# chaeyeongyun/VQ_SEG

Hardware: AMD Instinct MI355X
Metric: train images/sec @512x512 vqreptunet1x1 K=512 (higher is better)
Workload: dtype bf16; 1 GPU; CPS training iteration (2 x vqreptunet1x1, ResNet-50 encoder, K=[0,0,512,512,512], v1 recipe: 6 forwards + 4 backwards + 2 Adam steps) on 512x512x3 images -- BASELINE configs[2] (the metric's configuration): vqreptunet1x1 512x512, K = 512; labelled_per_gpu=32, unlabelled_per_gpu=32, parallelism=dp1, collectives=none (one process), conv_dtype=bf16

## Files before the change

include/vqseg.h:

```cpp
#ifndef VQSEG_H
#define VQSEG_H

#include <stddef.h>
#include <stdint.h>

#ifdef __cplusplus
extern "C" {
#endif

#define VQSEG_ABI_VERSION 1

#define VQSEG_EINVAL  (-1)
#define VQSEG_ENOSPC  (-2)
#define VQSEG_ENODEV  (-3)

int         vqseg_abi_version(void);
const char* vqseg_last_error(void);
const char* vqseg_kernel_name(const char* entry_point);

int vqseg_set_option(const char* key, int value);

int vqseg_profile_begin(int capacity);
int vqseg_profile_collect(int max_records, int64_t* n_rows_host, int* channels_host,
                          int* n_codes_host, float* ms_host,
                          int* kind_host );

int vqseg_conv_profile_begin(int capacity);
int vqseg_conv_profile_collect(int max_records, double* flops_host, int* kind_host, float* ms_host,
                               int* shape_host );

size_t vqseg_vq_workspace_bytes(int64_t n_rows, int channels, int n_codes);
int vqseg_vq_forward_f32(const float* x, const float* codebook, const void* prepared,
                         int64_t n_rows, int channels, int n_codes, int training,
                         float commitment_weight, float* quant, int64_t* idx, float* loss,
                         float* dead_pct, float* dmin, void* workspace, size_t workspace_bytes,
                         void* stream);

int vqseg_vq_forward_group(int n_levels, int bf16, const void* const* x, const float* const* codebook,
                           const void* const* prepared, const int64_t* n_rows, const int* channels, const int* n_codes,
                           int training, const float* commitment_weight, void* const* quant, int64_t* const* idx,
                           float* const* loss, float* const* dead_pct, void* const* workspace,
                           const size_t* workspace_bytes, void* stream);

size_t vqseg_vq_filter_counter_offset(int64_t n_rows, int channels, int n_codes);

int vqseg_vq_tiles_per_wave(int n_levels, const int64_t* n_rows_host, const int* n_codes_host);

int vqseg_vq_assign_f32(const float* x, const float* codebook, const void* prepared,
                        int64_t n_rows, int channels, int n_codes, int64_t* idx, float* dmin,
                        void* workspace, size_t workspace_bytes, void* stream);
int vqseg_vq_assign_bf16(const void* x, const float* codebook, const void* prepared,
                         int64_t n_rows, int channels, int n_codes, int64_t* idx, float* dmin,
                         void* workspace, size_t workspace_bytes, void* stream);

int vqseg_vq_assign_s3(const void* x, const float* codebook, const void* prepared,
                       int64_t n_rows, int channels, int n_codes, int64_t* idx, float* dmin,
                       void* workspace, size_t workspace_bytes, void* stream);

size_t vqseg_vq_prepared_bytes(int channels, int n_codes);
int vqseg_vq_prepare_f32(const float* codebook, int channels, int n_codes, void* prepared,
                         size_t prepared_bytes, void* stream);

int vqseg_vq_backward_f32(const float* grad_quant, const float* grad_loss, const float* x,
                          const float* quant, int64_t n_rows, int channels,
                          float commitment_weight, float* grad_x, void* stream);

int vqseg_vq_forward_bf16(const void* x, const float* codebook, const void* prepared, int64_t n_rows, int channels,
                          int n_codes, int training, float commitment_weight, void* quant, int64_t* idx, float* loss,
                          float* dead_pct, float* dmin, void* workspace, size_t workspace_bytes, void* stream);
int vqseg_vq_backward_bf16(const void* grad_quant, const float* grad_loss, const void* x, const int64_t* idx,
                           const float* codebook, int64_t n_rows, int channels, float commitment_weight,
                           void* grad_x, void* stream);

size_t vqseg_kmeans_workspace_bytes(int64_t n_rows, int channels, int n_codes);
int vqseg_kmeans_f32(const float* samples, float* means, int64_t* bins, int64_t n_rows,
                     int channels, int n_codes, int iters, void* workspace,
                     size_t workspace_bytes, void* stream);
int vqseg_kmeans_accumulate_f32(const float* samples, const float* means, int64_t n_rows,
                                int channels, int n_codes, float* sums, int64_t* counts,
                                void* workspace, size_t workspace_bytes, void* stream);
int vqseg_kmeans_finalize_f32(const float* sums, const int64_t* counts, float* means,
                              int channels, int n_codes, void* stream);


int vqseg_vq_code_sums(int bf16, const void* x, const int64_t* idx, int64_t n_rows, int channels, int n_codes,
                       float* sums, int64_t* counts, void* workspace, size_t workspace_bytes, void* stream);
int vqseg_vq_ema_update_f32(float* cluster_size, float* embed_avg, float* codebook, const float* sums,
                            const int64_t* counts, int channels, int n_codes, float decay, float eps, float* scratch,
                            void* stream);
int vqseg_vq_revive_candidates(int bf16, const void* x, int64_t n_rows, int channels, int n_codes, uint64_t seed,
                               const int64_t* counter, int rank, int world, float* cand, float* ok, void* stream);
int vqseg_vq_ema_update_revive_f32(float* cluster_size, float* embed_avg, float* codebook, const float* sums,
                                   const int64_t* counts, int channels, int n_codes, float decay, float eps, float* scratch,
                                   const float* cand, const float* ok, float threshold, int64_t* counter, int64_t* revived,
                                   void* stream);


size_t vqseg_conv_packed_elems(int cout, int cin, int kh, int kw, int transpose_flip);
int vqseg_conv_pack_weights_f32(const float* w, int cout, int cin, int kh, int kw, int transpose_flip,
                                void* hi, void* lo, void* stream);

int64_t vqseg_conv_stat_slots(int64_t m_rows, int cout);
int vqseg_conv2d_f(const void* x, const void* x2, int c1, const void* w_hi, const void* w_lo, void* y,
                   float* stat_partial, int n, int h, int w, int cin, int cout, int kh, int kw, int stride,
                   int pad, int reflect, int up, int ho, int wo, int precise, void* stream);

int vqseg_conv2d_affine_f(const void* x, const void* x2, int c1, const void* w_hi, const void* w_lo,
                          const float* scale, const float* shift, const void* res, int relu, void* y,
                          int n, int h, int w, int cin, int cout, int kh, int kw, int stride, int pad, int reflect,
                          int ho, int wo, int precise, void* stream);
int vqseg_conv2d_affine_bits_f(const void* x, const void* w_hi, const float* scale, const float* shift, const void* res,
                               const unsigned char* res_bits, void* y, int n, int h, int w, int cin, int cout, int kh, int kw,
                               int pad, int ho, int wo, void* stream);

size_t vqseg_conv2d_wgrad_workspace_bytes(int n, int h, int w, int cin, int ho, int wo, int cout, int kh, int kw);
int vqseg_conv2d_wgrad_f(const void* gy, const void* x, const void* x2, int c1, int n, int h, int w, int cin,
                         int ho, int wo, int cout, int kh, int kw, int stride, int pad, int reflect, int precise,
                         int cin_out, int im2col, int accumulate, void* workspace, size_t workspace_bytes, float* gw,
                         void* stream);
int vqseg_conv2d_wgrad2_f(const void* gy, const void* x, const void* x2, int n, const void* gy_b, const void* x_b, const void* x2_b,
                          int n_b, int c1, int h, int w, int cin, int ho, int wo, int cout, int kh, int kw, int stride, int pad,
                          int reflect, int precise, int cin_out, int im2col, int accumulate, void* workspace, size_t workspace_bytes,
                          float* gw, void* stream);

int vqseg_bn_sync_ints(int c);
int vqseg_bn_finalize_f(float* partial, int64_t m_rows, int c, const float* gamma, const float* beta,
                        float* run_mean, float* run_var, float momentum, float eps, int training,
                        float* scale, float* shift, float* save_mean, float* save_invstd,
                        int64_t* num_batches_tracked , int* sync, void* stream);
int vqseg_bn_apply_f(int bf16, const void* y, const void* res, const float* scale, const float* shift,
                     int64_t m_rows, int c, int relu, void* out, void* stream);
size_t vqseg_bn_backward_workspace_floats(int64_t m_rows, int c);
int vqseg_bn_backward_f(int bf16, const void* g_out, const void* out, const void* y, const float* mean,
                        const float* invstd, const float* gamma, const float* fwd_scale, const float* fwd_shift,
                        int64_t m_rows, int c, int relu, int training, int accumulate,
                        float* workspace, float* dgamma, float* dbeta, void* g_y, void* g_res, int* sync, void* stream);
int vqseg_bn_apply_bits_f(const void* y, const void* res, const float* scale, const float* shift, int64_t m_rows, int c,
                          void* out, unsigned char* bits, void* stream);
int vqseg_bn_backward_bits_f(const void* g_out, const unsigned char* bits, const void* y, const float* mean,
                             const float* invstd, const float* gamma, int64_t m_rows, int c, int training, int accumulate,
                             float* workspace, float* dgamma, float* dbeta, void* g_y, void* g_res, int* sync, void* stream);

int vqseg_maxpool3x3s2_f(int bf16, int backward, const void* x, const void* g, int n, int h, int w, int c,
                         void* out, unsigned char* idx, void* stream);

int vqseg_bilinear_f(int bf16, int backward, const void* src, int n, int h, int w, int c, int ho, int wo,
                     int align_corners, void* dst, void* stream);

int vqseg_head1x1_forward_f(int bf16, const void* x, const float* w, int64_t m_rows, int cin, int cout,
                            float* y, void* stream);
size_t vqseg_head1x1_backward_workspace_floats(int64_t m_rows, int cin, int cout);
int vqseg_head1x1_backward_f(int bf16, const void* x, const float* w, const float* g, int64_t m_rows, int cin,
                             int cout, void* gx, float* gw, float* workspace, void* stream);
int vqseg_head1x1_backward_add_f(int bf16, const void* x, const float* w, const float* g, int64_t m_rows, int cin,
                                 int cout, void* gx, float* gw, float* workspace, const void* gx_add, void* stream);
int vqseg_maxpool3x3s2_backward_add_f(int bf16, const void* g, const unsigned char* idx, const void* gx_add, int n, int h, int w,
                                      int c, void* gx, void* stream);

int vqseg_im2col_f(int out_bf16, const float* x, int n, int h, int w, int cin, int kh, int kw, int stride,
                   int pad, int reflect, int ho, int wo, int kp, void* out, void* stream);
int vqseg_reflect_fold_f(int bf16, const void* gp, int n, int h, int w, int c, void* gx, void* stream);
int vqseg_stem7_conv_f(int s3, const float* x, const void* w_img, void* y, float* stat_partial, const float* scale, const float* shift, int relu,
                       int n, int h, int w, int reflect, void* stream);
int vqseg_reflect_ring_f(const void* gy, const void* t_hi, void* ring, void* gx, int n, int h, int w, int cgy, int cgx, void* stream);

int vqseg_conv_pack_weights_s3_f32(const float* w, int cout, int cin, int c1, int kh, int kw, void* out, void* stream);

int vqseg_conv_pack_all_f32(const float* w, int cout, int cin, int k, int c1, void* fwd, void* tr, void* s3, void* stream);
size_t vqseg_conv_packed_s2_elems(int cout, int cin, int k);
int vqseg_conv_pack_weights_s2_f32(const float* w, int cout, int cin, int k, void* hi, void* lo, void* stream);
int vqseg_conv2d_dgrad_s2_f(const void* gy, const void* w_hi, const void* w_lo, void* gx, int n, int ho, int wo, int cout, int cin,
                            int k, int oh, int ow, int precise, int accumulate, void* stream);
int64_t vqseg_conv2d_dgrad_s2_fold_rows(int n, int h, int w, int reflect);
int vqseg_conv2d_dgrad_s2_fold_f(const void* gy, const void* w_hi, void* gx, int n, int ho, int wo, int cout, int cin, int h, int w,
                                 int reflect, void* stream);
int vqseg_s3_split_f(const float* x, int64_t rows, int channels, void* y, void* stream);
int vqseg_s3_merge_f(const void* x, int64_t rows, int channels, float* y, void* stream);
int vqseg_s3_maxpool3x3s2_f(const void* x, int n, int h, int w, int c, void* y, void* stream);
int vqseg_s3_bilinear_f(const void* x, int n, int h, int w, int c, int ho, int wo, int align_corners, void* y, void* stream);
int vqseg_cast_f(int to_bf16, const void* x, int64_t n, void* y, void* stream);

size_t vqseg_proto_loss_workspace_bytes(int64_t m_rows, int c, int k);
int vqseg_proto_loss_forward_f(int bf16, const void* x, const float* proto, const int64_t* labels,
                               const unsigned char* keep, const float* conf, int64_t m_rows, int c, int k,
                               int variant, float scale, float margin, int easy_margin,
                               void* workspace, size_t workspace_bytes, double* loss, void* stream);
int vqseg_proto_loss_backward_f(int bf16, const void* x, const float* proto, const int64_t* labels,
                                const unsigned char* keep, const float* conf, int64_t m_rows, int c, int k,
                                int variant, float scale, float margin, int easy_margin, const float* g_loss,
                                void* gx, float* gproto, void* workspace, size_t workspace_bytes, void* stream);

size_t vqseg_dice_workspace_bytes(int b, int c, int64_t hw);
int vqseg_dice_sums_forward_f(const float* logits, int64_t stride_b, int64_t stride_c, int64_t stride_px,
                              const int64_t* target, int b, int c, int64_t hw, int64_t ignore_index,
                              void* workspace, size_t workspace_bytes, float* inter, float* sets, void* stream);
int vqseg_dice_sums_backward_f(const float* logits, int64_t stride_b, int64_t stride_c, int64_t stride_px,
                               const int64_t* target, int b, int c, int64_t hw, int64_t ignore_index,
                               const float* g_inter, const float* g_sets, float* g_logits, void* stream);

int vqseg_dice_ce_sums_forward_f(const float* logits, int64_t stride_b, int64_t stride_c, int64_t stride_px,
                                 const int64_t* target, int b, int c, int64_t hw, int64_t ignore_index,
                                 void* workspace, size_t workspace_bytes, float* inter, float* sets, float* ce,
                                 void* stream);
int vqseg_dice_ce_sums_backward_f(const float* logits, int64_t stride_b, int64_t stride_c, int64_t stride_px,
                                  const int64_t* target, int b, int c, int64_t hw, int64_t ignore_index,
                                  const float* g_inter, const float* g_sets, const float* g_ce, float* g_logits,
                                  void* stream);

int vqseg_softmax_stats_f(const float* logits, int64_t stride_b, int64_t stride_c, int64_t stride_px, int b, int c,
                          int64_t hw, int64_t* label, float* entropy, float* top, void* stream);

int vqseg_confusion_counts_f(const float* logits, int64_t stride_b, int64_t stride_c, int64_t stride_px,
                             const int64_t* target, int b, int c, int64_t hw, int64_t* counts, void* stream);

size_t vqseg_focal_workspace_bytes(int b, int64_t hw);
int vqseg_focal_forward_f(const float* logits, int64_t stride_b, int64_t stride_c, int64_t stride_px,
                          const int64_t* target, int b, int c, int64_t hw, int64_t ignore_index, const float* weight,
                          float alpha, float gamma, int pre_softmax, void* workspace, size_t workspace_bytes,
                          double* per_image, float* loss2, float* loss_map, void* stream);
int vqseg_focal_backward_f(const float* logits, int64_t stride_b, int64_t stride_c, int64_t stride_px,
                           const int64_t* target, int b, int c, int64_t hw, int64_t ignore_index, const float* weight,
                           float alpha, float gamma, int pre_softmax, const float* g_scalar, float scale,
                           const float* g_map, float* g_logits, void* stream);

int vqseg_wce_sums_forward_f(const float* logits, int64_t stride_b, int64_t stride_c, int64_t stride_px,
                             const int64_t* target, int b, int c, int64_t hw, int64_t ignore_index, const float* weight,
                             void* workspace, size_t workspace_bytes, float* ce, void* stream);
int vqseg_wce_sums_backward_f(const float* logits, int64_t stride_b, int64_t stride_c, int64_t stride_px,
                              const int64_t* target, int b, int c, int64_t hw, int64_t ignore_index, const float* weight,
                              const float* g_ce, float* g_logits, void* stream);

int vqseg_class_weight_f(const int64_t* labels, int64_t n, int num_classes, int64_t* counts, float* weight, void* stream);

int vqseg_cps_loss_combine_f(int n_sup, int n_cps, int c, const float* const* inter, const float* const* sets, const float* const* ce,
                             const int* b, float cps_weight, float ce_weight, float eps, const float* const* commit, int n_commit,
                             int levels, float commit_weight, const double* const* proto, int n_proto, float proto_weight,
                             float* const* g_inter, float* const* g_sets, float* const* g_ce, float* out, void* stream);
size_t vqseg_order_stats_workspace_bytes(void);
int vqseg_order_stats_f(const float* x, int64_t n, int64_t k, void* workspace, size_t workspace_bytes, float* out2,
                        void* stream);

#define VQSEG_ADAM_CHUNK 4096
typedef struct VqsegAdamParam {
    float* p;
    const float* g;
    float* m;
    float* v;
    int64_t numel;
    int32_t k, cout, cin, c1;
    void* fwd;
    void* tr;
    void* s3;
} VqsegAdamParam;
int64_t vqseg_adam_work_items(int64_t numel, int k, int cout, int cin);
int vqseg_adam_step_f32(const VqsegAdamParam* params_dev, const int32_t* items_dev, int n_items, double lr, double beta1,
                        double beta2, double eps, int64_t step, void* stream);

typedef struct VqsegEmaParam {
    float* e;
    int32_t copy;
    int32_t reserved;
    void* fwd;
    void* tr;
    void* s3;
} VqsegEmaParam;
int vqseg_adam_ema_step_f32(const VqsegAdamParam* params_dev, const VqsegEmaParam* ema_dev, const int32_t* items_dev, int n_items,
                            double lr, double beta1, double beta2, double eps, int64_t step, double ema_decay, int copy_all,
                            void* stream);

int vqseg_batch_u8_f(int n, const uint8_t* img_cache, const uint8_t* mask_cache, const int64_t* img_offsets_host,
                     const int64_t* mask_offsets_host, int h, int w, int mh, int mw, const float* f32_lut, const int64_t* label_lut,
                     float* img_out, uint8_t* target_out, int64_t* label_out, void* stream);

int vqseg_box_mix_f(int mode, int elem_bytes, const void* src, void* out, int n, int planes, int h, int w, int64_t stride_s,
                    int64_t stride_p, int64_t stride_px, const int32_t* boxes_host, uint64_t fill_bits, void* stream);

int vqseg_affine_warp_f(int mode, int elem_bytes, const void* src, void* out, int n, int planes, int h, int w, int64_t src_stride_s,
                        int64_t out_stride_s, int64_t stride_p, int64_t stride_px, const float* matrices_host, uint64_t fill_bits,
                        void* stream);

int vqseg_resize_argmax_f(const float* const* views_host, const int* flips_host, int n_views, int64_t stride_b, int64_t stride_c,
                          int64_t stride_px, int b, int c, int h, int w, int ho, int wo, uint8_t* label, float* top,
                          const int64_t* target, int64_t* counts, void* stream);

#define VQSEG_BLEND_UNIFORM 0
#define VQSEG_BLEND_LINEAR 1
int vqseg_extract_windows_f(const float* images, int64_t stride_b, int64_t stride_c, int64_t stride_px, int b, int h, int w, int wh, int ww,
                            int sy, int sx, int nh, int nw, const int* flips_host, int n_flips, float* out, void* stream);
int vqseg_merge_argmax_f(const float* const* views_host, const int* flips_host, int n_views, int64_t stride_b, int64_t stride_c,
                         int64_t stride_px, int b, int c, int lh, int lw, int ho, int wo, int wh, int ww, int sy, int sx, int blend,
                         uint8_t* label, float* top, const int64_t* target, int64_t* counts, void* stream);

int vqseg_render_sheet_u8(const float* image, int64_t stride_b, int64_t stride_c, int64_t stride_px, int h, int w, const uint8_t* pred,
                          const int64_t* target, int ht, int wt, int b, int ho, int wo, int c, const int* kinds_host, const int* x0_host,
                          const int* width_host, int n_panels, const float* palette_f_host, const uint8_t* palette_u8_host,
                          const float* fill_f_host, const uint8_t* fill_u8_host, float alpha, int box2, uint8_t* canvas, int64_t pitch,
                          int rows, int cols, void* stream);

size_t vqseg_supcon_workspace_bytes(int64_t hw);
int vqseg_supcon_forward_f(int bf16, const void* f1, const void* f2, int64_t row_stride, int h, int w, int c, const int64_t* gt1,
                           const int64_t* gt2, int ht, int wt, float temperature, void* workspace, size_t workspace_bytes, float* out,
                           void* stream);
int vqseg_supcon_backward_f(int bf16, const void* f1, const void* f2, int64_t row_stride, int h, int w, int c, const int64_t* gt1,
                            const int64_t* gt2, int ht, int wt, float temperature, const float* stats, const float* g_scalar, void* d_f1,
                            void* d_f2, int64_t grad_row_stride, void* stream);

#ifdef __cplusplus
}
#endif
#endif
```

vq_seg_amd/_hip.py:

```python
from __future__ import annotations

import ctypes
import os
from ctypes import c_char_p, c_double, c_float, c_int, c_int64, c_size_t, c_void_p
from typing import Optional, Tuple

import numpy as np
import torch

_HERE = os.path.dirname(os.path.abspath(__file__))
LIB_PATH = os.environ.get("VQSEG_LIB") or os.path.join(_HERE, "libvqseg_hip.so")

SYMBOLS = {
    "vqseg_abi_version": (c_int, []),
    "vqseg_last_error": (c_char_p, []),
    "vqseg_kernel_name": (c_char_p, [c_char_p]),
    "vqseg_set_option": (c_int, [c_char_p, c_int]),
    "vqseg_profile_begin": (c_int, [c_int]),
    "vqseg_profile_collect": (c_int, [c_int, c_void_p, c_void_p, c_void_p, c_void_p, c_void_p]),
    "vqseg_conv_profile_begin": (c_int, [c_int]),
    "vqseg_conv_profile_collect": (c_int, [c_int, c_void_p, c_void_p, c_void_p, c_void_p]),
    "vqseg_vq_workspace_bytes": (c_size_t, [c_int64, c_int, c_int]),
    "vqseg_vq_filter_counter_offset": (c_size_t, [c_int64, c_int, c_int]),
    "vqseg_vq_tiles_per_wave": (c_int, [c_int, c_void_p, c_void_p]),
    "vqseg_vq_forward_f32": (c_int, [c_void_p, c_void_p, c_void_p, c_int64, c_int, c_int, c_int, c_float, c_void_p,
                                     c_void_p, c_void_p, c_void_p, c_void_p, c_void_p, c_size_t, c_void_p]),
    "vqseg_vq_forward_bf16": (c_int, [c_void_p, c_void_p, c_void_p, c_int64, c_int, c_int, c_int, c_float, c_void_p,
                                      c_void_p, c_void_p, c_void_p, c_void_p, c_void_p, c_size_t, c_void_p]),
    "vqseg_vq_forward_group": (c_int, [c_int, c_int] + [c_void_p] * 6 + [c_int, c_void_p] + [c_void_p] * 6 + [c_void_p]),
    "vqseg_vq_backward_bf16": (c_int, [c_void_p, c_void_p, c_void_p, c_void_p, c_void_p, c_int64, c_int, c_float, c_void_p, c_void_p]),
    "vqseg_vq_assign_f32": (c_int, [c_void_p, c_void_p, c_void_p, c_int64, c_int, c_int, c_void_p, c_void_p, c_void_p,
                                    c_size_t, c_void_p]),
    "vqseg_vq_assign_bf16": (c_int, [c_void_p, c_void_p, c_void_p, c_int64, c_int, c_int, c_void_p, c_void_p, c_void_p,
                                     c_size_t, c_void_p]),
    "vqseg_vq_assign_s3": (c_int, [c_void_p, c_void_p, c_void_p, c_int64, c_int, c_int, c_void_p, c_void_p, c_void_p,
                                   c_size_t, c_void_p]),
    "vqseg_vq_prepared_bytes": (c_size_t, [c_int, c_int]),
    "vqseg_vq_prepare_f32": (c_int, [c_void_p, c_int, c_int, c_void_p, c_size_t, c_void_p]),
    "vqseg_vq_backward_f32": (c_int, [c_void_p, c_void_p, c_void_p, c_void_p, c_int64, c_int, c_float, c_void_p,
                                      c_void_p]),
    "vqseg_kmeans_workspace_bytes": (c_size_t, [c_int64, c_int, c_int]),
    "vqseg_kmeans_f32": (c_int, [c_void_p, c_void_p, c_void_p, c_int64, c_int, c_int, c_int, c_void_p, c_size_t,
                                 c_void_p]),
    "vqseg_kmeans_accumulate_f32": (c_int, [c_void_p, c_void_p, c_int64, c_int, c_int, c_void_p, c_void_p, c_void_p,
                                            c_size_t, c_void_p]),
    "vqseg_kmeans_finalize_f32": (c_int, [c_void_p, c_void_p, c_void_p, c_int, c_int, c_void_p]),
    "vqseg_vq_code_sums": (c_int, [c_int, c_void_p, c_void_p, c_int64, c_int, c_int, c_void_p, c_void_p, c_void_p, c_size_t, c_void_p]),
    "vqseg_vq_ema_update_f32": (c_int, [c_void_p, c_void_p, c_void_p, c_void_p, c_void_p, c_int, c_int, c_float, c_float, c_void_p,
                                        c_void_p]),
    "vqseg_vq_revive_candidates": (c_int, [c_int, c_void_p, c_int64, c_int, c_int, ctypes.c_uint64, c_void_p, c_int, c_int, c_void_p, c_void_p,
                                           c_void_p]),
    "vqseg_vq_ema_update_revive_f32": (c_int, [c_void_p, c_void_p, c_void_p, c_void_p, c_void_p, c_int, c_int, c_float, c_float, c_void_p,
                                               c_void_p, c_void_p, c_float, c_void_p, c_void_p, c_void_p]),
    "vqseg_conv_packed_elems": (c_size_t, [c_int] * 5),
    "vqseg_conv_pack_weights_f32": (c_int, [c_void_p] + [c_int] * 5 + [c_void_p, c_void_p, c_void_p]),
    "vqseg_conv_stat_slots": (c_int64, [c_int64, c_int]),
    "vqseg_conv2d_f": (c_int, [c_void_p, c_void_p, c_int, c_void_p, c_void_p, c_void_p, c_void_p] + [c_int] * 14 + [c_void_p]),
    "vqseg_conv2d_affine_f": (c_int, [c_void_p, c_void_p, c_int, c_void_p, c_void_p, c_void_p, c_void_p, c_void_p, c_int, c_void_p] +
                              [c_int] * 13 + [c_void_p]),
    "vqseg_conv2d_wgrad_workspace_bytes": (c_size_t, [c_int] * 9),
    "vqseg_conv2d_wgrad_f": (c_int, [c_void_p, c_void_p, c_void_p] + [c_int] * 17 + [c_void_p, c_size_t, c_void_p, c_void_p]),
    "vqseg_conv2d_wgrad2_f": (c_int, [c_void_p, c_void_p, c_void_p, c_int, c_void_p, c_void_p, c_void_p, c_int] + [c_int] * 16 +
                              [c_void_p, c_size_t, c_void_p, c_void_p]),
    "vqseg_bn_sync_ints": (c_int, [c_int]),
    "vqseg_bn_finalize_f": (c_int, [c_void_p, c_int64, c_int, c_void_p, c_void_p, c_void_p, c_void_p, c_float, c_float, c_int,
                                   c_void_p, c_void_p, c_void_p, c_void_p, c_void_p, c_void_p, c_void_p]),
    "vqseg_bn_apply_f": (c_int, [c_int, c_void_p, c_void_p, c_void_p, c_void_p, c_int64, c_int, c_int, c_void_p, c_void_p]),
    "vqseg_bn_backward_workspace_floats": (c_size_t, [c_int64, c_int]),
    "vqseg_bn_backward_f": (c_int, [c_int] + [c_void_p] * 8 + [c_int64, c_int, c_int, c_int, c_int] + [c_void_p] * 7),
    "vqseg_conv2d_affine_bits_f": (c_int, [c_void_p] * 7 + [c_int] * 10 + [c_void_p]),
    "vqseg_bn_apply_bits_f": (c_int, [c_void_p] * 4 + [c_int64, c_int, c_void_p, c_void_p, c_void_p]),
    "vqseg_bn_backward_bits_f": (c_int, [c_void_p] * 6 + [c_int64, c_int, c_int, c_int] + [c_void_p] * 7),
    "vqseg_maxpool3x3s2_f": (c_int, [c_int, c_int, c_void_p, c_void_p, c_int, c_int, c_int, c_int, c_void_p, c_void_p, c_void_p]),
    "vqseg_bilinear_f": (c_int, [c_int, c_int, c_void_p] + [c_int] * 7 + [c_void_p, c_void_p]),
    "vqseg_head1x1_forward_f": (c_int, [c_int, c_void_p, c_void_p, c_int64, c_int, c_int, c_void_p, c_void_p]),
    "vqseg_head1x1_backward_workspace_floats": (c_size_t, [c_int64, c_int, c_int]),
    "vqseg_head1x1_backward_f": (c_int, [c_int, c_void_p, c_void_p, c_void_p, c_int64, c_int, c_int, c_void_p, c_void_p,
                                        c_void_p, c_void_p]),
    "vqseg_proto_loss_workspace_bytes": (c_size_t, [c_int64, c_int, c_int]),
    "vqseg_proto_loss_forward_f": (c_int, [c_int, c_void_p, c_void_p, c_void_p, c_void_p, c_void_p, c_int64, c_int, c_int, c_int,
                                           c_float, c_float, c_int, c_void_p, c_size_t, c_void_p, c_void_p]),
    "vqseg_proto_loss_backward_f": (c_int, [c_int, c_void_p, c_void_p, c_void_p, c_void_p, c_void_p, c_int64, c_int, c_int, c_int,
                                            c_float, c_float, c_int, c_void_p, c_void_p, c_void_p, c_void_p, c_size_t, c_void_p]),
    "vqseg_dice_workspace_bytes": (c_size_t, [c_int, c_int, c_int64]),
    "vqseg_dice_sums_forward_f": (c_int, [c_void_p, c_int64, c_int64, c_int64, c_void_p, c_int, c_int, c_int64, c_int64, c_void_p, c_size_t,
                                          c_void_p, c_void_p, c_void_p]),
    "vqseg_dice_sums_backward_f": (c_int, [c_void_p, c_int64, c_int64, c_int64, c_void_p, c_int, c_int, c_int64, c_int64, c_void_p,
                                           c_void_p, c_void_p, c_void_p]),
    "vqseg_dice_ce_sums_forward_f": (c_int, [c_void_p, c_int64, c_int64, c_int64, c_void_p, c_int, c_int, c_int64, c_int64, c_void_p,
                                             c_size_t, c_void_p, c_void_p, c_void_p, c_void_p]),
    "vqseg_dice_ce_sums_backward_f": (c_int, [c_void_p, c_int64, c_int64, c_int64, c_void_p, c_int, c_int, c_int64, c_int64, c_void_p,
                                              c_void_p, c_void_p, c_void_p, c_void_p]),
    "vqseg_focal_workspace_bytes": (c_size_t, [c_int, c_int64]),
    "vqseg_focal_forward_f": (c_int, [c_void_p, c_int64, c_int64, c_int64, c_void_p, c_int, c_int, c_int64, c_int64, c_void_p, c_float, c_float,
                                      c_int, c_void_p, c_size_t, c_void_p, c_void_p, c_void_p, c_void_p]),
    "vqseg_focal_backward_f": (c_int, [c_void_p, c_int64, c_int64, c_int64, c_void_p, c_int, c_int, c_int64, c_int64, c_void_p, c_float, c_float,
                                       c_int, c_void_p, c_float, c_void_p, c_void_p, c_void_p]),
    "vqseg_wce_sums_forward_f": (c_int, [c_void_p, c_int64, c_int64, c_int64, c_void_p, c_int, c_int, c_int64, c_int64, c_void_p, c_void_p,
                                         c_size_t, c_void_p, c_void_p]),
    "vqseg_wce_sums_backward_f": (c_int, [c_void_p, c_int64, c_int64, c_int64, c_void_p, c_int, c_int, c_int64, c_int64, c_void_p, c_void_p,
                                          c_void_p, c_void_p]),
    "vqseg_class_weight_f": (c_int, [c_void_p, c_int64, c_int, c_void_p, c_void_p, c_void_p]),
    "vqseg_softmax_stats_f": (c_int, [c_void_p, c_int64, c_int64, c_int64, c_int, c_int, c_int64, c_void_p, c_void_p, c_void_p, c_void_p]),
    "vqseg_confusion_counts_f": (c_int, [c_void_p, c_int64, c_int64, c_int64, c_void_p, c_int, c_int, c_int64, c_void_p, c_void_p]),
    "vqseg_order_stats_workspace_bytes": (c_size_t, []),
    "vqseg_order_stats_f": (c_int, [c_void_p, c_int64, c_int64, c_void_p, c_size_t, c_void_p, c_void_p]),
    "vqseg_im2col_f": (c_int, [c_int, c_void_p] + [c_int] * 12 + [c_void_p, c_void_p]),
    "vqseg_reflect_fold_f": (c_int, [c_int, c_void_p, c_int, c_int, c_int, c_int, c_void_p, c_void_p]),
    "vqseg_reflect_ring_f": (c_int, [c_void_p, c_void_p, c_void_p, c_void_p, c_int, c_int, c_int, c_int, c_int, c_void_p]),
    "vqseg_cast_f": (c_int, [c_int, c_void_p, c_int64, c_void_p, c_void_p]),
    "vqseg_conv_pack_all_f32": (c_int, [c_void_p, c_int, c_int, c_int, c_int, c_void_p, c_void_p, c_void_p, c_void_p]),
    "vqseg_conv_packed_s2_elems": (c_size_t, [c_int, c_int, c_int]),
    "vqseg_conv_pack_weights_s2_f32": (c_int, [c_void_p, c_int, c_int, c_int, c_void_p, c_void_p, c_void_p]),
    "vqseg_conv2d_dgrad_s2_f": (c_int, [c_void_p, c_void_p, c_void_p, c_void_p] + [c_int] * 10 + [c_void_p]),
    "vqseg_stem7_conv_f": (c_int, [c_int, c_void_p, c_void_p, c_void_p, c_void_p, c_void_p, c_void_p] + [c_int] * 5 + [c_void_p]),
    "vqseg_conv2d_dgrad_s2_fold_rows": (ctypes.c_int64, [c_int] * 4),
    "vqseg_cps_loss_combine_f": (c_int, [c_int, c_int, c_int, c_void_p, c_void_p, c_void_p, c_void_p, c_float, c_float, c_float, c_void_p, c_int, c_int,
                                         c_float, c_void_p, c_int, c_float, c_void_p, c_void_p, c_void_p, c_void_p, c_void_p]),
    "vqseg_conv2d_dgrad_s2_fold_f": (c_int, [c_void_p, c_void_p, c_void_p] + [c_int] * 8 + [c_void_p]),
    "vqseg_head1x1_backward_add_f": (c_int, [c_int, c_void_p, c_void_p, c_void_p, c_int64, c_int, c_int, c_void_p, c_void_p,
                                            c_void_p, c_void_p, c_void_p]),
    "vqseg_maxpool3x3s2_backward_add_f": (c_int, [c_int, c_void_p, c_void_p, c_void_p, c_int, c_int, c_int, c_int, c_void_p, c_void_p]),
    "vqseg_conv_pack_weights_s3_f32": (c_int, [c_void_p] + [c_int] * 5 + [c_void_p, c_void_p]),
    "vqseg_s3_split_f": (c_int, [c_void_p, c_int64, c_int, c_void_p, c_void_p]),
    "vqseg_s3_merge_f": (c_int, [c_void_p, c_int64, c_int, c_void_p, c_void_p]),
    "vqseg_s3_maxpool3x3s2_f": (c_int, [c_void_p, c_int, c_int, c_int, c_int, c_void_p, c_void_p]),
    "vqseg_s3_bilinear_f": (c_int, [c_void_p] + [c_int] * 7 + [c_void_p, c_void_p]),
    "vqseg_adam_work_items": (c_int64, [c_int64, c_int, c_int, c_int]),
    "vqseg_adam_step_f32": (c_int, [c_void_p, c_void_p, c_int, c_double, c_double, c_double, c_double, c_int64, c_void_p]),
    "vqseg_adam_ema_step_f32": (c_int, [c_void_p, c_void_p, c_void_p, c_int, c_double, c_double, c_double, c_double, c_int64, c_double, c_int,
                                        c_void_p]),
    "vqseg_batch_u8_f": (c_int, [c_int, c_void_p, c_void_p, c_void_p, c_void_p] + [c_int] * 4 + [c_void_p] * 6),
    "vqseg_box_mix_f": (c_int, [c_int, c_int, c_void_p, c_void_p] + [c_int] * 4 + [c_int64] * 3 + [c_void_p, ctypes.c_uint64, c_void_p]),
    "vqseg_affine_warp_f": (c_int, [c_int, c_int, c_void_p, c_void_p] + [c_int] * 4 + [c_int64] * 4 + [c_void_p, ctypes.c_uint64, c_void_p]),
    "vqseg_resize_argmax_f": (c_int, [c_void_p, c_void_p, c_int] + [c_int64] * 3 + [c_int] * 6 + [c_void_p] * 5),
    "vqseg_extract_windows_f": (c_int, [c_void_p] + [c_int64] * 3 + [c_int] * 9 + [c_void_p, c_int, c_void_p, c_void_p]),
    "vqseg_merge_argmax_f": (c_int, [c_void_p, c_void_p, c_int] + [c_int64] * 3 + [c_int] * 11 + [c_void_p] * 5),
    "vqseg_render_sheet_u8": (c_int, [c_void_p] + [c_int64] * 3 + [c_int] * 2 + [c_void_p] * 2 + [c_int] * 6 + [c_void_p] * 3 + [c_int] +
                              [c_void_p] * 4 + [c_float, c_int, c_void_p, c_int64, c_int, c_int, c_void_p]),
    "vqseg_supcon_workspace_bytes": (c_size_t, [c_int64]),
    "vqseg_supcon_forward_f": (c_int, [c_int, c_void_p, c_void_p, c_int64, c_int, c_int, c_int, c_void_p, c_void_p, c_int, c_int, c_float,
                                       c_void_p, c_size_t, c_void_p, c_void_p]),
    "vqseg_supcon_backward_f": (c_int, [c_int, c_void_p, c_void_p, c_int64, c_int, c_int, c_int, c_void_p, c_void_p, c_int, c_int, c_float,
                                        c_void_p, c_void_p, c_void_p, c_void_p, c_int64, c_void_p]),
}

_lib: Optional[ctypes.CDLL] = None


class HipLibraryError(RuntimeError):
    pass


def _bind_symbols(handle: ctypes.CDLL) -> ctypes.CDLL:
    for name, (res, args) in SYMBOLS.items():
        fn = getattr(handle, name)
        fn.restype, fn.argtypes = res, args
    return handle


def lib() -> ctypes.CDLL:
    global _lib
    if _lib is None:
        if not os.path.exists(LIB_PATH):
            raise HipLibraryError(
                f"{LIB_PATH} not found: build it with `python -c 'import __graft_entry__ as g; g.build()'` "
                f"(or `make -C vq_seg_amd/csrc`). There is no CPU fallback.")
        handle = _bind_symbols(ctypes.CDLL(LIB_PATH))
        if handle.vqseg_abi_version() != 1:
            raise HipLibraryError("libvqseg_hip.so ABI version mismatch")
        for kv in filter(None, os.environ.get("VQSEG_OPTS", "").split(",")):
            key, _, val = kv.partition("=")
            if key.strip().startswith("py_"):
                PY_OPTS[key.strip()] = int(val)
                continue
            if handle.vqseg_set_option(key.strip().encode(), int(val)) < 0:
                raise HipLibraryError(f"VQSEG_OPTS: unknown option {key!r}")
        _lib = handle
    return _lib


PY_OPTS: dict = {}
FILTER_DIAG = None


_BF_DTYPE = {0: torch.float32, 1: torch.bfloat16, 2: torch.bfloat16}


def tptr(t, name: str, dtype=None, numel: Optional[int] = None, bf: Optional[int] = None, at_least: bool = False, dense: bool = True):
    if t is None:
        return None
    if bf is not None:
        dtype = _BF_DTYPE[bf]
    try:
        if (dtype is None or t.dtype is dtype or (type(dtype) is tuple and t.dtype in dtype)) and t.is_cuda and \
                (numel is None or (t.numel() >= numel if at_least else t.numel() == numel)) and \
                (not dense or t.is_contiguous() or (t.dim() == 4 and t.is_contiguous(memory_format=torch.channels_last))):
            return t.data_ptr()
    except AttributeError:
        pass
    return _tptr_report(t, name, dtype, numel, at_least, dense)


def _tptr_report(t, name, dtype, numel, at_least, dense):
    def bad(msg):
        return HipLibraryError(f"{name}: {msg}")
    if not isinstance(t, torch.Tensor):
        raise bad(f"expected a tensor, got {type(t).__name__}")
    if dtype is not None and (t.dtype not in dtype if isinstance(dtype, tuple) else t.dtype != dtype):
        if dense:
            raise bad(f"expected {dtype}, got {t.dtype}")
        names = " or ".join(str(d).removeprefix("torch.") for d in (dtype if isinstance(dtype, tuple) else (dtype,)))
        raise bad(f"expected a {names} tensor, got {t.dtype}")
    if dense and not t.is_contiguous() and not (t.dim() == 4 and t.is_contiguous(memory_format=torch.channels_last)):
        raise bad(f"expected a dense (contiguous) tensor, got strides {tuple(t.stride())} for shape {tuple(t.shape)}")
    if numel is not None and (t.numel() < numel if at_least else t.numel() != numel):
        raise bad(f"the sizes passed along need {'at least ' if at_least else ''}{numel} elements, the tensor has {t.numel()} (shape {tuple(t.shape)})")
    if not t.is_cuda:
        return _NotOnGpu(f"{name}: the HIP path needs a tensor on a 'cuda' (ROCm) device; got {t.device}. There is no CPU fallback.")
    return t.data_ptr()


class _NotOnGpu:
    __slots__ = ("msg",)

    def __init__(self, msg: str):
        self.msg = msg

    def __add__(self, _offset):
        return self


def on_gpu(ptr):
    if type(ptr) is _NotOnGpu:
        raise HipLibraryError(ptr.msg)
    return ptr


def _dev(t: torch.Tensor, dtype: torch.dtype, name: str, numel: Optional[int] = None):
    if t is None:
        raise HipLibraryError(f"{name}: expected a tensor, got None")
    return tptr(t, name, dtype=dtype, numel=numel)


def _stream() -> int:
    return torch.cuda.current_stream().cuda_stream


def _failed(L, name: str, rc: int) -> HipLibraryError:
    return HipLibraryError(f"{name} failed (code {rc}): {L.vqseg_last_error().decode(errors='replace')}")


def launch(name: str, dev, *args, handle=None) -> None:
    L = handle or lib()
    if type(dev) is not torch.device:
        dev = torch.device(dev)
    if dev.type == "cuda":
        try:
            with torch.cuda.device(dev):
                rc = getattr(L, name)(*args, _stream())
        except ctypes.ArgumentError:
            for a in args:
                on_gpu(a)
            raise
        if rc != 0:
            raise _failed(L, name, rc)
        return
    for a in args:
        on_gpu(a)
    raise HipLibraryError(f"{name}: the HIP path needs tensors on a 'cuda' (ROCm) device; got {dev}. There is no CPU fallback.")


def _workspace(nbytes: int, device) -> torch.Tensor:
    return torch.empty(int(nbytes), dtype=torch.uint8, device=device)


def vq_prepare(codebook: torch.Tensor) -> torch.Tensor:
    L = lib()
    k, c = codebook.shape
    wp = _dev(codebook, torch.float32, "codebook")
    nbytes = L.vqseg_vq_prepared_bytes(c, k)
    blob = _workspace(nbytes, codebook.device)
    launch("vqseg_vq_prepare_f32", codebook.device, wp, c, k, blob.data_ptr(), nbytes)
    return blob


def vq_forward(rows: torch.Tensor, codebook: torch.Tensor, training: bool, commitment_weight: float,
               want_dmin: bool = False, prepared: Optional[torch.Tensor] = None):
    L = lib()
    n, c = rows.shape
    k = codebook.shape[0]
    bf16 = rows.dtype == torch.bfloat16
    xp, wp = tptr(rows, "rows", bf=int(bf16), numel=n * c), _dev(codebook, torch.float32, "codebook", k * c)
    dev = rows.device
    quant = torch.empty_like(rows)
    idx = torch.empty(n, dtype=torch.int64, device=dev)
    scal = torch.empty(2, dtype=torch.float32, device=dev)
    dmin = torch.empty(n, dtype=torch.float32, device=dev) if want_dmin else None
    nbytes = L.vqseg_vq_workspace_bytes(n, c, k)
    ws = _workspace(nbytes, dev)
    launch("vqseg_vq_forward_bf16" if bf16 else "vqseg_vq_forward_f32", dev, xp, wp,
           tptr(prepared, "prepared codebook", dtype=torch.uint8, numel=L.vqseg_vq_prepared_bytes(c, k)), n, c, k,
           int(bool(training)), float(commitment_weight), quant.data_ptr(), idx.data_ptr(), scal.data_ptr(), scal.data_ptr() + 4,
           dmin.data_ptr() if want_dmin else None, ws.data_ptr(), nbytes)
    out = (quant, idx, scal[0:1], scal[1])
    return out + (dmin,) if want_dmin else out


def bind(path: str) -> ctypes.CDLL:
    return _bind_symbols(ctypes.CDLL(path))


def vq_forward_group(rows_list, codebooks, prepared_list, training: bool, commitment_weights, handle=None, s3: bool = False):
    L = handle or lib()
    nl = len(rows_list)
    bf16 = 2 if s3 else int(rows_list[0].dtype == torch.bfloat16)
    if s3 and training:
        raise HipLibraryError("vq_forward_group: split-3 rows are an eval-mode format (training must be False)")
    dev = rows_list[0].device
    ptr = lambda ps: (c_void_p * nl)(*map(on_gpu, ps))
    ns = np.array([r.shape[0] for r in rows_list], dtype=np.int64)
    cs = np.array([w.shape[1] for w in codebooks], dtype=np.int32)
    ks = np.array([w.shape[0] for w in codebooks], dtype=np.int32)
    cw = np.array([float(w) for w in commitment_weights], dtype=np.float32)
    xs, wps, preps, quants, idxs, scals, wss = [], [], [], [], [], [], []
    for r, w in zip(rows_list, codebooks):
        if r.dtype != rows_list[0].dtype:
            raise HipLibraryError("vq_forward_group: one row type per call")
        if w.dim() != 2 or r.dim() != 2 or r.shape[1] != (2 if s3 else 1) * w.shape[1]:
            raise HipLibraryError(f"vq_forward_group: rows {tuple(r.shape)} do not match a codebook {tuple(w.shape)}" + (" (split-3 rows: 2C columns)" if s3 else ""))
        xs.append(tptr(r, "rows", bf=bf16, numel=r.shape[0] * r.shape[1]))
        wps.append(_dev(w, torch.float32, "codebook", w.shape[0] * w.shape[1]))
        quants.append(torch.empty_like(r))
        idxs.append(torch.empty(r.shape[0], dtype=torch.int64, device=dev))
        scals.append(torch.empty(2, dtype=torch.float32, device=dev))
        wss.append(_workspace(L.vqseg_vq_workspace_bytes(r.shape[0], w.shape[1], w.shape[0]), dev))
    for w, p_ in zip(codebooks, prepared_list):
        preps.append(tptr(p_, "prepared codebook", dtype=torch.uint8, numel=L.vqseg_vq_prepared_bytes(w.shape[1], w.shape[0])))
    wsb = (c_size_t * nl)(*[w.numel() for w in wss])
    launch("vqseg_vq_forward_group", dev, nl, bf16, ptr(xs), ptr(wps), ptr(preps), ns.ctypes.data, cs.ctypes.data, ks.ctypes.data,
           int(bool(training)), cw.ctypes.data, ptr(q.data_ptr() for q in quants), ptr(i.data_ptr() for i in idxs),
           ptr(s.data_ptr() for s in scals), ptr(s.data_ptr() + 4 for s in scals), ptr(w.data_ptr() for w in wss),
           ctypes.cast(wsb, c_void_p), handle=handle)
    if FILTER_DIAG is not None and bf16:
        for r, w, ws_ in zip(rows_list, codebooks, wss):
            off = L.vqseg_vq_filter_counter_offset(r.shape[0], w.shape[1], w.shape[0])
            FILTER_DIAG.append((r.shape[0], w.shape[1], w.shape[0], ws_[off:off + 256].view(torch.int32) if off else None))
    return [(q, i, s[0:1], s[1]) for q, i, s in zip(quants, idxs, scals)]


def set_option(key: str, value: int) -> int:
    prev = lib().vqseg_set_option(key.encode(), int(value))
    if prev < 0:
        raise HipLibraryError(f"vqseg_set_option: unknown option {key!r} or bad value {value}")
    return prev


def vq_tiles_per_wave(n_rows, n_codes) -> int:
    rows = [n_rows] if isinstance(n_rows, int) else list(n_rows)
    codes = [n_codes] if isinstance(n_codes, int) else list(n_codes)
    if len(rows) != len(codes):
        raise ValueError("vq_tiles_per_wave: one code count per row count")
    t = lib().vqseg_vq_tiles_per_wave(len(rows), (ctypes.c_int64 * len(rows))(*rows), (c_int * len(codes))(*codes))
    if t < 0:
        raise _failed(lib(), "vqseg_vq_tiles_per_wave", t)
    return t


def vq_assign(rows: torch.Tensor, codebook: torch.Tensor, want_dmin: bool = False,
              prepared: Optional[torch.Tensor] = None, want_filter_count: bool = False, s3: bool = False, want_filter_state: bool = False):
    L = lib()
    n, c = rows.shape
    k = codebook.shape[0]
    bf16 = rows.dtype == torch.bfloat16
    if s3:
        if c != 2 * codebook.shape[1]:
            raise HipLibraryError(f"vq_assign: split-3 rows {tuple(rows.shape)} do not match a codebook {tuple(codebook.shape)} (2C columns)")
        c //= 2
    xp, wp = tptr(rows, "rows", bf=2 if s3 else int(bf16), numel=n * c * (2 if s3 else 1)), _dev(codebook, torch.float32, "codebook", k * c)
    dev = rows.device
    idx = torch.empty(n, dtype=torch.int64, device=dev)
    dmin = torch.empty(n, dtype=torch.float32, device=dev) if want_dmin else None
    nbytes = L.vqseg_vq_workspace_bytes(n, c, k)
    ws = _workspace(nbytes, dev)
    launch("vqseg_vq_assign_s3" if s3 else "vqseg_vq_assign_bf16" if bf16 else "vqseg_vq_assign_f32", dev, xp, wp,
           tptr(prepared, "prepared codebook", dtype=torch.uint8, numel=L.vqseg_vq_prepared_bytes(c, k)), n, c, k,
           idx.data_ptr(), dmin.data_ptr() if want_dmin else None, ws.data_ptr(), nbytes)
    if want_filter_count:
        off = L.vqseg_vq_filter_counter_offset(n, c, k) if bf16 else 0
        amb = ws[off:off + 256].view(torch.int32).sum() if off else None
        return (idx, dmin, amb) if want_dmin else (idx, amb)
    if want_filter_state:
        off = L.vqseg_vq_filter_counter_offset(n, c, k) if bf16 else 0
        state = ws[off:off + 260].view(torch.int32).clone() if off else None
        return (idx, dmin, state) if want_dmin else (idx, state)
    return (idx, dmin) if want_dmin else idx


def vq_backward(grad_quant: torch.Tensor, grad_loss: Optional[torch.Tensor], rows: torch.Tensor, quant: torch.Tensor,
                commitment_weight: float) -> torch.Tensor:
    n, c = rows.shape
    gq = _dev(grad_quant, torch.float32, "grad_quant", n * c)
    gl = _dev(grad_loss, torch.float32, "grad_loss", 1) if grad_loss is not None else None
    gx = torch.empty_like(rows)
    launch("vqseg_vq_backward_f32", rows.device, gq, gl, _dev(rows, torch.float32, "rows", n * c), _dev(quant, torch.float32, "quant", n * c),
           n, c, float(commitment_weight), gx.data_ptr())
    return gx


def vq_backward_bf16(grad_quant: torch.Tensor, grad_loss: Optional[torch.Tensor], rows: torch.Tensor, idx: torch.Tensor,
                     codebook: torch.Tensor, commitment_weight: float) -> torch.Tensor:
    n, c = rows.shape
    gq = _dev(grad_quant, torch.bfloat16, "grad_quant", n * c)
    gl = _dev(grad_loss, torch.float32, "grad_loss", 1) if grad_loss is not None else None
    gx = torch.empty_like(rows)
    if codebook.dim() != 2 or codebook.shape[1] != c:
        raise HipLibraryError(f"codebook: expected (K, {c}), got {tuple(codebook.shape)}")
    launch("vqseg_vq_backward_bf16", rows.device, gq, gl, _dev(rows, torch.bfloat16, "rows", n * c), _dev(idx, torch.int64, "idx", n),
           _dev(codebook, torch.float32, "codebook"), n, c, float(commitment_weight), gx.data_ptr())
    return gx


def kmeans(samples: torch.Tensor, means: torch.Tensor, iters: int) -> Tuple[torch.Tensor, torch.Tensor]:
    L = lib()
    n, c = samples.shape
    k = means.shape[0]
    sp, mp = _dev(samples, torch.float32, "samples", n * c), _dev(means, torch.float32, "means", k * c)
    bins = torch.zeros(k, dtype=torch.int64, device=samples.device)
    nbytes = L.vqseg_kmeans_workspace_bytes(n, c, k)
    ws = _workspace(nbytes, samples.device)
    launch("vqseg_kmeans_f32", samples.device, sp, mp, bins.data_ptr(), n, c, k, int(iters), ws.data_ptr(), nbytes)
    return means, bins


def kmeans_accumulate(samples: torch.Tensor, means: torch.Tensor) -> Tuple[torch.Tensor, torch.Tensor]:
    L = lib()
    n, c = samples.shape
    k = means.shape[0]
    sp, mp = _dev(samples, torch.float32, "samples", n * c), _dev(means, torch.float32, "means", k * c)
    sums = torch.empty(k, c, dtype=torch.float32, device=samples.device)
    counts = torch.empty(k, dtype=torch.int64, device=samples.device)
    nbytes = L.vqseg_kmeans_workspace_bytes(n, c, k)
    ws = _workspace(nbytes, samples.device)
    launch("vqseg_kmeans_accumulate_f32", samples.device, sp, mp, n, c, k, sums.data_ptr(), counts.data_ptr(), ws.data_ptr(), nbytes)
    return sums, counts


def kmeans_finalize(sums: torch.Tensor, counts: torch.Tensor, means: torch.Tensor) -> torch.Tensor:
    k, c = means.shape
    launch("vqseg_kmeans_finalize_f32", means.device, _dev(sums, torch.float32, "sums", k * c), _dev(counts, torch.int64, "counts", k),
           _dev(means, torch.float32, "means", k * c), c, k)
    return means


def vq_code_sums(rows: torch.Tensor, idx: torch.Tensor, k: int, out: Optional[torch.Tensor] = None) -> Tuple[torch.Tensor, torch.Tensor]:
    L = lib()
    n, c = rows.shape
    if rows.dtype not in (torch.float32, torch.bfloat16):
        raise HipLibraryError(f"rows: expected torch.float32 or torch.bfloat16, got {rows.dtype}")
    ip = _dev(idx, torch.int64, "idx", n)
    sums = torch.empty(k, c, dtype=torch.float32, device=rows.device) if out is None else out
    counts = torch.empty(k, dtype=torch.int64, device=rows.device)
    nbytes = L.vqseg_kmeans_workspace_bytes(n, c, k)
    ws = _workspace(nbytes, rows.device)
    bf = int(rows.dtype == torch.bfloat16)
    launch("vqseg_vq_code_sums", rows.device, bf, tptr(rows, "rows", bf=bf, numel=n * c), ip, n, c, k,
           sums.data_ptr() if out is None else _dev(out, torch.float32, "out", k * c), counts.data_ptr(), ws.data_ptr(), nbytes)
    return sums, counts


def vq_revive_candidates(rows: torch.Tensor, seed: int, counter: torch.Tensor, k: int, rank: int, world: int, out=None):
    n, c = rows.shape
    if rows.dtype not in (torch.float32, torch.bfloat16):
        raise HipLibraryError(f"rows: expected torch.float32 or torch.bfloat16, got {rows.dtype}")
    bf = int(rows.dtype == torch.bfloat16)
    xp, tp = tptr(rows, "rows", bf=bf, numel=n * c), _dev(counter, torch.int64, "counter", 1)
    if out is None:
        out = (torch.empty(k, c, dtype=torch.float32, device=rows.device), torch.empty(k, dtype=torch.float32, device=rows.device))
    cand, ok = out
    launch("vqseg_vq_revive_candidates", rows.device, bf, xp, n, c, k, int(seed) & 0xFFFFFFFFFFFFFFFF, tp, int(rank), int(world),
           _dev(cand, torch.float32, "candidates", k * c), _dev(ok, torch.float32, "ok", k))
    return cand, ok


def vq_ema_update(cluster_size: torch.Tensor, embed_avg: torch.Tensor, codebook: torch.Tensor, sums: torch.Tensor,
                  counts: torch.Tensor, decay: float, eps: float, candidates: Optional[torch.Tensor] = None,
                  ok: Optional[torch.Tensor] = None, threshold: float = 0.0, counter: Optional[torch.Tensor] = None,
                  revived: Optional[torch.Tensor] = None) -> None:
    k, c = codebook.shape
    if cluster_size.shape != (k,) or embed_avg.shape != (k, c) or sums.shape != (k, c) or counts.shape != (k,):
        raise ValueError("vq_ema_update: shapes must be (K,), (K, C), (K, C), (K, C), (K,)")
    if threshold == 0:
        scratch = torch.empty(1, dtype=torch.float32, device=codebook.device)
        launch("vqseg_vq_ema_update_f32", codebook.device, _dev(cluster_size, torch.float32, "cluster_size"),
               _dev(embed_avg, torch.float32, "embed_avg"), _dev(codebook, torch.float32, "codebook"), _dev(sums, torch.float32, "sums"),
               _dev(counts, torch.int64, "counts"), c, k, float(decay), float(eps), scratch.data_ptr())
        return
    scratch = torch.empty(1 + k, dtype=torch.float32, device=codebook.device)
    launch("vqseg_vq_ema_update_revive_f32", codebook.device, _dev(cluster_size, torch.float32, "cluster_size"),
           _dev(embed_avg, torch.float32, "embed_avg"), _dev(codebook, torch.float32, "codebook"), _dev(sums, torch.float32, "sums"),
           _dev(counts, torch.int64, "counts"), c, k, float(decay), float(eps), scratch.data_ptr(),
           _dev(candidates, torch.float32, "candidates", k * c), _dev(ok, torch.float32, "ok", k), float(threshold),
           _dev(counter, torch.int64, "counter", 1), _dev(revived, torch.int64, "revived", 1))


def batch_u8(img_cache: torch.Tensor, img_offsets, hw: Tuple[int, int], f32_lut: torch.Tensor, img_out: torch.Tensor,
             mask_cache: Optional[torch.Tensor] = None, mask_offsets=None, mask_hw: Tuple[int, int] = (0, 0),
             label_lut: Optional[torch.Tensor] = None, target_out: Optional[torch.Tensor] = None,
             label_out: Optional[torch.Tensor] = None) -> None:
    n = len(img_offsets)
    (h, w), (mh, mw) = hw, mask_hw
    io = np.ascontiguousarray(img_offsets, dtype=np.int64)
    mo = np.ascontiguousarray(mask_offsets, dtype=np.int64) if mask_offsets is not None else None
    if n and (int(io.min()) < 0 or int(io.max()) + h * w * 3 > img_cache.numel()):
        raise HipLibraryError("batch_u8: an image offset lies outside the image cache")
    if mask_cache is not None:
        if mo is None or len(mo) != n:
            raise HipLibraryError("batch_u8: one mask offset per sample required")
        if n and (int(mo.min()) < 0 or int(mo.max()) + mh * mw > mask_cache.numel()):
            raise HipLibraryError("batch_u8: a mask offset lies outside the mask cache")
    if img_out.dim() != 4 or not img_out.is_contiguous(memory_format=torch.channels_last):
        raise HipLibraryError("batch_u8: img_out must be a channels_last (n, 3, h, w) tensor")
    launch("vqseg_batch_u8_f", img_out.device, n, tptr(img_cache, "img_cache", dtype=torch.uint8), tptr(mask_cache, "mask_cache", dtype=torch.uint8),
           io.ctypes.data, mo.ctypes.data if mo is not None else None, h, w, mh, mw,
           tptr(f32_lut, "f32_lut", dtype=torch.float32, numel=256), tptr(label_lut, "label_lut", dtype=torch.int64, numel=256),
           tptr(img_out, "img_out", dtype=torch.float32, numel=n * 3 * h * w),
           tptr(target_out, "target_out", dtype=torch.uint8, numel=n * mh * mw),
           tptr(label_out, "label_out", dtype=torch.int64, numel=n * mh * mw))


BOX_MIX_DTYPES = (torch.uint8, torch.bfloat16, torch.float32, torch.int64)
BOX_MIX_CALLS = 0


def box_mix(src: torch.Tensor, boxes, mode: str = "mix", fill=0, out: Optional[torch.Tensor] = None) -> torch.Tensor:
    global BOX_MIX_CALLS
    if mode not in ("mix", "fill"):
        raise HipLibraryError(f"box_mix: mode must be 'mix' or 'fill', got {mode!r}")
    if not isinstance(src, torch.Tensor) or src.dim() not in (3, 4):
        raise HipLibraryError("box_mix: src must be a (n, P, h, w) or (n, h, w) tensor")
    n, (h, w) = src.shape[0], src.shape[-2:]
    planes = src.shape[1] if src.dim() == 4 else 1
    bx = np.ascontiguousarray(boxes, dtype=np.int32)
    if bx.shape != (n, 4):
        raise HipLibraryError(f"box_mix: one (y1, x1, cut_h, cut_w) box per sample required: {n} samples, boxes of shape {bx.shape}")
    if n and (int(bx.min()) < 0 or int((bx[:, 0] + bx[:, 2]).max()) > h or int((bx[:, 1] + bx[:, 3]).max()) > w):
        raise HipLibraryError(f"box_mix: a box lies outside the {h} x {w} image")
    if out is None:
        out = torch.empty_like(src)
    elif not isinstance(out, torch.Tensor) or out.shape != src.shape or out.stride() != src.stride():
        raise HipLibraryError("box_mix: out must have src's shape and layout")
    numel = n * planes * h * w
    sp, op = tptr(src, "src", dtype=BOX_MIX_DTYPES, numel=numel), tptr(out, "out", dtype=src.dtype, numel=numel)
    if numel == 0:
        raise HipLibraryError("box_mix: empty tensor")
    strides = (planes * h * w, h * w, 1) if src.is_contiguous() else (planes * h * w, 1, planes)
    bits = int.from_bytes(torch.tensor([fill], dtype=src.dtype).view(torch.uint8).numpy().tobytes(), "little") if mode == "fill" else 0
    launch("vqseg_box_mix_f", src.device, int(mode == "fill"), src.element_size(), sp, op, n, planes, h, w, *strides, bx.ctypes.data, bits)
    BOX_MIX_CALLS += 1
    return out


AFFINE_WARP_BILINEAR_DTYPES = (torch.float32, torch.bfloat16)
AFFINE_WARP_NEAREST_DTYPES = (torch.uint8, torch.int8, torch.bool, torch.int16, torch.bfloat16, torch.float16, torch.int32, torch.float32, torch.int64,
                              torch.float64)
AFFINE_WARP_CALLS = 0


def affine_warp(src: torch.Tensor, matrices, mode: str = "bilinear", fill=0, out: Optional[torch.Tensor] = None) -> torch.Tensor:
    global AFFINE_WARP_CALLS
    if mode not in ("bilinear", "nearest"):
        raise HipLibraryError(f"affine_warp: mode must be 'bilinear' or 'nearest', got {mode!r}")
    if not isinstance(src, torch.Tensor) or src.dim() not in (3, 4):
        raise HipLibraryError("affine_warp: src must be a (n, P, h, w) or (n, h, w) tensor")
    n, (h, w) = src.shape[0], src.shape[-2:]
    planes = src.shape[1] if src.dim() == 4 else 1
    try:
        mats = np.ascontiguousarray(matrices, dtype=np.float32)
    except (TypeError, ValueError):
        raise HipLibraryError("affine_warp: matrices must be n rows of six numbers") from None
    if mats.shape != (n, 6):
        raise HipLibraryError(f"affine_warp: one (M00, M01, 0, M10, M11, 0) row per sample required: {n} samples, matrices of shape {mats.shape}")
    if not np.isfinite(mats).all():
        raise HipLibraryError("affine_warp: a matrix entry is not finite")
    if mats[:, (2, 5)].any():
        raise HipLibraryError("affine_warp: the translation slots (entries 2 and 5 of a row) are reserved and must be 0")
    dtypes = AFFINE_WARP_BILINEAR_DTYPES if mode == "bilinear" else AFFINE_WARP_NEAREST_DTYPES
    numel = n * planes * h * w
    sp = tptr(src, "src", dtype=dtypes, numel=numel)
    if numel == 0:
        raise HipLibraryError("affine_warp: empty tensor")
    planar = src.is_contiguous()
    inner = (h * w, 1) if planar else (1, planes)
    out_stride = planes * h * w
    if out is None:
        out = torch.empty_like(src)
        op = tptr(out, "out", dtype=src.dtype, numel=numel)
    else:
        if not isinstance(out, torch.Tensor) or out.shape != src.shape:
            raise HipLibraryError("affine_warp: out must have src's shape and layout")
        one = out[:1]
        if (one.is_contiguous() if planar else (one.dim() == 4 and one.is_contiguous(memory_format=torch.channels_last))) and \
                (n == 1 or out.stride(0) >= out_stride):
            out_stride = out.stride(0) if n > 1 else out_stride
        else:
            raise HipLibraryError("affine_warp: out must have src's shape and layout")
        op = tptr(out, "out", dtype=src.dtype, numel=numel, dense=False)
        if type(sp) is int and type(op) is int and sp == op:
            raise HipLibraryError("affine_warp: out of place only")
    bits = int.from_bytes(torch.tensor([fill], dtype=src.dtype).view(torch.uint8).numpy().tobytes(), "little") if mode == "nearest" else 0
    launch("vqseg_affine_warp_f", src.device, int(mode == "nearest"), src.element_size(), sp, op, n, planes, h, w, planes * h * w, out_stride,
           *inner, mats.ctypes.data, bits)
    AFFINE_WARP_CALLS += 1
    return out


RENDER_KINDS = {"image": 0, "target": 1, "pred": 2, "detail": 3, "mix_pred": 4, "mix_detail": 5, "fill": 6}
RENDER_SHEET_CALLS = 0


def render_sheet(canvas: torch.Tensor, panels, size, num_classes: int, palette, fill=(1.0, 1.0, 1.0), image: Optional[torch.Tensor] = None,
                 pred: Optional[torch.Tensor] = None, target: Optional[torch.Tensor] = None, alpha: float = 0.4, box2: bool = False,
                 cols: Optional[int] = None) -> torch.Tensor:
    global RENDER_SHEET_CALLS
    E = HipLibraryError
    b, ho, wo = (int(v) for v in size)
    c = int(num_classes)
    rows = b * ho
    if not isinstance(canvas, torch.Tensor) or canvas.dim() != 3 or canvas.shape[2] != 3:
        raise E("render_sheet: canvas must be a (rows, cols, 3) uint8 tensor")
    orows, ocols = int(canvas.shape[0]), int(canvas.shape[1])
    cols = ocols * (2 if box2 else 1) if cols is None else int(cols)
    if box2 and (rows % 2 or cols % 2):
        raise E(f"render_sheet: box2 needs a sheet of even height and width, got {rows} x {cols}")
    if (orows, ocols) != ((rows // 2, cols // 2) if box2 else (rows, cols)):
        raise E(f"render_sheet: a {rows} x {cols} sheet{' halved by box2' if box2 else ''} needs a canvas of "
                f"{(rows // 2, cols // 2) if box2 else (rows, cols)} pixels, got {(orows, ocols)}")
    if orows == 0 or ocols == 0:
        raise E("render_sheet: empty canvas")
    if canvas.stride(2) != 1 or (ocols > 1 and canvas.stride(1) != 3) or (orows > 1 and canvas.stride(0) < 3 * ocols):
        raise E(f"render_sheet: canvas pixels must be dense RGB bytes with rows at least a row apart, got strides {tuple(canvas.stride())}")
    pitch = canvas.stride(0) if orows > 1 else 3 * ocols
    rows_ = [(RENDER_KINDS.get(k, -1) if isinstance(k, str) else int(k), int(x), int(wd)) for k, x, wd in panels]
    if any(k < 0 for k, _, _ in rows_):
        raise E(f"render_sheet: panel kinds are {sorted(RENDER_KINDS)}, got {[p[0] for p in panels]}")
    pal = np.ascontiguousarray(palette, dtype=np.float64)
    if pal.shape != (2 * c + 1, 3):
        raise E(f"render_sheet: the palette of {c} classes has {2 * c + 1} rows of 3 (class, wrong, ignore), got shape {pal.shape}")
    fil = np.ascontiguousarray(fill, dtype=np.float64).reshape(-1)
    if fil.shape != (3,):
        raise E("render_sheet: fill is one RGB colour")
    pal_f, fil_f = pal.astype(np.float32), fil.astype(np.float32)
    pal_u, fil_u = (np.floor(np.clip(a, 0.0, 1.0) * 255.0).astype(np.uint8) for a in (pal, fil))
    ip = pp = tp = None
    strides, (h, w), (ht, wt) = (0, 0, 0), (0, 0), (0, 0)
    if image is not None:
        if not isinstance(image, torch.Tensor) or image.dim() != 4 or image.shape[0] != b or image.shape[1] != 3:
            raise E(f"render_sheet: image must be a ({b}, 3, h, w) tensor")
        h, w = int(image.shape[2]), int(image.shape[3])
        ip = tptr(image, "image", dtype=torch.float32, numel=b * 3 * h * w)
        strides = (3 * h * w, h * w, 1) if image.is_contiguous() else (3 * h * w, 1, 3)
    if pred is not None:
        if not isinstance(pred, torch.Tensor) or tuple(pred.shape) != (b, ho, wo):
            raise E(f"render_sheet: pred must have the shape {(b, ho, wo)}, got {tuple(getattr(pred, 'shape', ()))}")
        pp = tptr(pred, "pred", dtype=torch.uint8, numel=b * ho * wo)
    if target is not None:
        if not isinstance(target, torch.Tensor) or target.dim() != 3 or target.shape[0] != b:
            raise E(f"render_sheet: target must be a ({b}, ht, wt) tensor")
        ht, wt = int(target.shape[1]), int(target.shape[2])
        tp = tptr(target, "target", dtype=torch.int64, numel=b * ht * wt)
    cp = tptr(canvas, "canvas", dtype=torch.uint8, numel=orows * ocols * 3, dense=False)
    arr = np.ascontiguousarray(rows_, dtype=np.int32).reshape(-1, 3).T.copy()
    launch("vqseg_render_sheet_u8", canvas.device, ip, *strides, h, w, pp, tp, ht, wt, b, ho, wo, c, arr[0].ctypes.data, arr[1].ctypes.data,
           arr[2].ctypes.data, len(rows_), pal_f.ctypes.data, pal_u.ctypes.data, fil_f.ctypes.data, fil_u.ctypes.data, float(alpha), int(bool(box2)),
           cp, pitch, rows, cols)
    RENDER_SHEET_CALLS += 1
    return canvas


def _checked(name: str, *args, counts: bool = False) -> int:
    rc = getattr(lib(), name)(*args)
    if rc < 0 or (rc and not counts):
        raise _failed(lib(), name, rc)
    return rc


def profile_begin(capacity: int = 4096) -> None:
    _checked("vqseg_profile_begin", int(capacity))


def conv_profile_begin(capacity: int = 65536) -> None:
    _checked("vqseg_conv_profile_begin", int(capacity))


def conv_profile_collect(capacity: int = 65536, with_shape: bool = False):
    fl = np.zeros(capacity, dtype=np.float64)
    kd = np.zeros(capacity, dtype=np.int32)
    ms = np.zeros(capacity, dtype=np.float32)
    sh = np.zeros((capacity, 4), dtype=np.int32)
    cnt = _checked("vqseg_conv_profile_collect", capacity, fl.ctypes.data, kd.ctypes.data, ms.ctypes.data, sh.ctypes.data if with_shape else None, counts=True)
    if with_shape:
        return [(float(fl[i]), int(kd[i]), float(ms[i]), tuple(int(v) for v in sh[i])) for i in range(cnt)]
    return [(float(fl[i]), int(kd[i]), float(ms[i])) for i in range(cnt)]


def profile_collect(capacity: int = 4096, with_kind: bool = False):
    n = np.zeros(capacity, dtype=np.int64)
    c = np.zeros(capacity, dtype=np.int32)
    k = np.zeros(capacity, dtype=np.int32)
    ms = np.zeros(capacity, dtype=np.float32)
    kd = np.zeros(capacity, dtype=np.int32)
    cnt = _checked("vqseg_profile_collect", capacity, n.ctypes.data, c.ctypes.data, k.ctypes.data, ms.ctypes.data, kd.ctypes.data, counts=True)
    if with_kind:
        return [(int(n[i]), int(c[i]), int(k[i]), float(ms[i]), int(kd[i])) for i in range(cnt)]
    return [(int(n[i]), int(c[i]), int(k[i]), float(ms[i])) for i in range(cnt)]
```

vq_seg_amd/csrc/vq_host.hip:

```cpp
#include <hip/hip_runtime.h>
#include <stdint.h>

#include <vector>

#include "options.h"
#include "vq_internal.h"

namespace vqseg {

static inline int round_up(int v, int m) { return (v + m - 1) / m * m; }

static inline size_t up256(size_t v) { return (v + 255) & ~(size_t)255; }

static bool filter_shape_ok(int C, int K) { return K % 256 == 0 && C % 32 == 0 && K <= 65536; }

PreparedLayout prepared_layout(int C, int K) {
    const int Kp = round_up(K, 32);
    PreparedLayout l;
    l.off_e4 = 0;
    l.off_enorm = (size_t)C * Kp * sizeof(float);
    l.off_enmax = up256(l.off_enorm + (size_t)Kp * sizeof(float));
    l.off_eb = l.off_enmax + 256;
    l.bytes = filter_shape_ok(C, K) ? up256(l.off_eb + (size_t)2 * C * Kp * sizeof(unsigned short)) : l.off_eb;
    return l;
}

PreparedView prepared_view(const void* prepared, int C, int K) {
    const PreparedLayout l = prepared_layout(C, K);
    char* base = const_cast<char*>(static_cast<const char*>(prepared));
    return {reinterpret_cast<float*>(base + l.off_e4), reinterpret_cast<float*>(base + l.off_enorm),
            reinterpret_cast<float*>(base + l.off_enmax), reinterpret_cast<unsigned short*>(base + l.off_eb)};
}

size_t prepared_bytes(int C, int K) { return prepared_layout(C, K).bytes; }

static int g_vq_max_tiles = 8;
static int g_vq_fine_split = 1;
static int g_vq_bf16_filter = 1;
static int g_vq_filter_force_all = 0;
static int g_vq_filter_launches = 0;
static int g_vq_s3_filter = 1;
static const Option VQ_OPTIONS[] = {
    {"vq_max_tiles_per_wave", &g_vq_max_tiles, OPT_POW2_FAIL, 1, 8},
    {"vq_fine_split", &g_vq_fine_split, OPT_FLAG},
    {"vq_bf16_filter", &g_vq_bf16_filter, OPT_FLAG},
    {"vq_filter_force_all", &g_vq_filter_force_all, OPT_FLAG},
    {"vq_filter_launches", &g_vq_filter_launches},
    {"vq_s3_filter", &g_vq_s3_filter, OPT_FLAG},
};

int vq_set_option(const char* key, int value) { return apply_option(VQ_OPTIONS, key, value); }

VqPlan vq_plan(int64_t N, int C, int K) {
    VqPlan p;
    p.Cp = C;
    p.Kp = round_up(K, 32);
    size_t off = 0;
    p.off_prepared = off;
    off += prepared_bytes(C, K);
    p.off_keys = off;
    off += up256((size_t)N * sizeof(unsigned long long));
    p.off_hist = off;
    off += up256((size_t)p.Kp * sizeof(int));
    p.off_partial = off;
    off += (size_t)GATHER_BLOCKS_MAX * sizeof(float);
    off = up256(off);
    p.off_summary = p.off_brow = p.off_amb = p.off_pair_rc = off;
    p.pair_cap = 0;
    if (filter_shape_ok(C, K)) {
        p.off_summary = off;
        off += up256((size_t)N * (p.Kp / F_SUB) * sizeof(unsigned long long));
        p.off_brow = off;
        off += up256((size_t)N * sizeof(float));
        p.off_amb = off;
        off += 512;
        const long total_cap = 4 * N < (1L << 30) ? 4 * N : (1L << 30);
        p.pair_cap = (int)((total_cap + F_LISTS - 1) / F_LISTS);
        if (p.pair_cap < 1024) p.pair_cap = 1024;
        p.off_pair_rc = off;
        off += up256((size_t)p.pair_cap * F_LISTS * sizeof(unsigned long long));
    }
    p.bytes = up256(off);
    long blocks = (N + GATHER_ROWS_PER_BLOCK - 1) / GATHER_ROWS_PER_BLOCK;
    p.gather_blocks = (int)(blocks < GATHER_BLOCKS_MAX ? (blocks > 0 ? blocks : 1) : GATHER_BLOCKS_MAX);
    const int k1 = K;
    p.T = vq_group_tiles(1, &N, &k1);
    return p;
}

hipError_t launch_prepare(const float* W, int K, int C, void* prepared, hipStream_t st) {
    const int Kp = round_up(K, 32);
    const PreparedView pv = prepared_view(prepared, C, K);
    launch_prepare_exact(W, K, C, Kp, pv.E4, pv.enorm, st);
    if (filter_shape_ok(C, K)) launch_prepare_filter(W, K, C, Kp, pv.enorm, pv.Eb, pv.en_max, st);
    return hipGetLastError();
}

struct ProfShape {
    int64_t n;
    int c, k;
    int slot, group;
    int kind;
};
struct Profile {
    bool enabled = false;
    int capacity = 0;
    std::vector<hipEvent_t> ev;
    std::vector<ProfShape> shape;
};
static Profile g_prof;

hipError_t profile_begin(int capacity) {
    profile_release();
    g_prof.ev.resize((size_t)capacity * 2);
    for (auto& e : g_prof.ev) {
        hipError_t rc = hipEventCreate(&e);
        if (rc != hipSuccess) return rc;
    }
    g_prof.shape.clear();
    g_prof.capacity = capacity;
    g_prof.enabled = true;
    return hipSuccess;
}

void profile_release() {
    for (auto& e : g_prof.ev) (void)hipEventDestroy(e);
    g_prof.ev.clear();
    g_prof.shape.clear();
    g_prof.enabled = false;
    g_prof.capacity = 0;
}

int profile_collect(int max_records, int64_t* n, int* c, int* k, float* ms, int* kind) {
    g_prof.enabled = false;
    const int cnt = (int)g_prof.shape.size();
    int out = 0;
    for (int i = 0; i < cnt && out < max_records; ++i) {
        const ProfShape& sh = g_prof.shape[i];
        if (hipEventSynchronize(g_prof.ev[2 * sh.slot + 1]) != hipSuccess) break;
        float t = 0.f;
        if (hipEventElapsedTime(&t, g_prof.ev[2 * sh.slot], g_prof.ev[2 * sh.slot + 1]) != hipSuccess) break;
        double mine = 2.0 * (double)sh.n * sh.c * sh.k, all = 0.0;
        for (int j = sh.slot; j < sh.slot + sh.group && j < cnt; ++j) all += 2.0 * (double)g_prof.shape[j].n * g_prof.shape[j].c * g_prof.shape[j].k;
        n[out] = sh.n;
        c[out] = sh.c;
        k[out] = sh.k;
        ms[out] = (float)(t * (all > 0 ? mine / all : 1.0));
        if (kind) kind[out] = sh.kind;
        ++out;
    }
    profile_release();
    return out;
}


static unsigned assign_workgroups(int64_t N, int Kp, int T) {
    const long row_tiles = (N + ROWS_PER_WG - 1) / ROWS_PER_WG;
    return (unsigned)((row_tiles + 7) / 8 * 8 * (Kp / (32 * T)));
}

constexpr long VQ_FINE_WGS = 4096;
static long vq_group_wgs(int n, const int64_t* N, const int* K, int t) {
    long wgs = 0;
    for (int i = 0; i < n; ++i) {
        const int tiles = round_up(K[i], 32) / 32;
        if (tiles % t) return -1;
        wgs += ((N[i] + ROWS_PER_WG - 1) / ROWS_PER_WG) * (tiles / t);
    }
    return wgs;
}
int vq_group_tiles(int n, const int64_t* N, const int* K) {
    if (g_vq_fine_split)
        for (int t = g_vq_max_tiles; t >= 4; t >>= 1)
            if (vq_group_wgs(n, N, K, t) >= VQ_FINE_WGS) return t;
    for (int t = g_vq_max_tiles; t >= 1; t >>= 1) {
        const long wgs = vq_group_wgs(n, N, K, t);
        if (wgs >= 0 && (wgs >= 512 || t == 1)) return t;
    }
    return 1;
}

hipError_t launch_assign_group(int n, const void* const* x, int x_bf16, const int64_t* N, const int* C, const int* K,
                               const void* const* prepared, const VqPlan* plans, char* const* ws, int64_t* const* idx,
                               float* const* dmin, int T, hipStream_t st, const float* const* codebooks) {
    if (n < 1 || n > VQ_MAX_LEVELS) return hipErrorInvalidValue;
    int order[VQ_MAX_LEVELS];
    for (int i = 0; i < n; ++i) order[i] = i;
    for (int i = 0; i < n; ++i)
        for (int j = i + 1; j < n; ++j)
            if (C[order[j]] > C[order[i]]) { const int t = order[i]; order[i] = order[j]; order[j] = t; }
    bool filter = x_bf16 == VQ_ROWS_S3 ? g_vq_s3_filter != 0 : (x_bf16 && g_vq_bf16_filter);
    for (int i = 0; i < n; ++i) filter = filter && filter_shape_ok(C[i], K[i]);
    VqLevel lv[VQ_MAX_LEVELS];
    VqFilterGroup fg;
    fg.n = n;
    unsigned end = 0, fend = 0, rend = 0, send = 0, iend = 0;
    VqInitGroup ig;
    ig.n = n;
    for (int q = 0; q < n; ++q) {
        const int i = order[q];
        const PreparedView pv = prepared_view(prepared[i], C[i], K[i]);
        unsigned long long* keys = reinterpret_cast<unsigned long long*>(ws[i] + plans[i].off_keys);
        {
            long ib = (N[i] + 4095) / 4096;
            ib = ib < 1 ? 1 : (ib > 256 ? 256 : ib);
            iend += (unsigned)ib;
            ig.lv[q] = VqInitLevel{keys, (long)N[i], nullptr, reinterpret_cast<int*>(ws[i] + plans[i].off_hist), plans[i].Kp, iend};
        }
        end += assign_workgroups(N[i], plans[i].Kp, T);
        lv[q] = VqLevel{x[i], pv.E4, pv.enorm, keys, (long)N[i], C[i], plans[i].Kp, end};
        lv[q].K = K[i];
        if (filter) {
            int* amb = reinterpret_cast<int*>(ws[i] + plans[i].off_amb);
            ig.lv[q].amb = amb;
            lv[q].gate = amb + F_LISTS;
            lv[q].gate_cap = 0;
            const long row_tiles = (N[i] + F_ROWS - 1) / F_ROWS;
            fend += (unsigned)((row_tiles + 7) / 8 * 8 * (plans[i].Kp / F_CODES));
            rend += (unsigned)((N[i] + 255) / 256);
            {
                long per = (N[i] / 256 + F_LISTS - 1) / F_LISTS;
                if (per < 4) per = 4;
                if (per > 16) per = 16;
                send += (unsigned)(per * F_LISTS);
            }
            fg.lv[q] = VqFilterLevel{x[i], pv.Eb, pv.enorm, pv.en_max,
                                     reinterpret_cast<unsigned long long*>(ws[i] + plans[i].off_summary),
                                     reinterpret_cast<float*>(ws[i] + plans[i].off_brow),
                                     reinterpret_cast<unsigned long long*>(ws[i] + plans[i].off_pair_rc), amb, plans[i].pair_cap, keys,
                                     codebooks ? codebooks[i] : nullptr, pv.E4, (long)N[i], C[i], plans[i].Kp, fend, rend, send};
        }
    }
    launch_group_init(ig, st);
    const bool rec = g_prof.enabled && (int)g_prof.shape.size() + n <= g_prof.capacity;
    const size_t slot = g_prof.shape.size();
    if (rec) {
        for (int i = 0; i < n; ++i) g_prof.shape.push_back({N[i], C[i], K[i], (int)slot, n, filter ? 2 : (x_bf16 == VQ_ROWS_BF16 ? 1 : 0)});
        (void)hipEventRecord(g_prof.ev[2 * slot], st);
    }
    if (filter) {
        ++g_vq_filter_launches;
        launch_filter(fg, x_bf16, g_vq_filter_force_all, st);
    }
    launch_assign_levels(lv, n, T, x_bf16, st);
    if (rec) (void)hipEventRecord(g_prof.ev[2 * slot + 1], st);
    hipError_t e = hipGetLastError();
    if (e != hipSuccess) return e;
    for (int i = 0; i < n; ++i) {
        launch_unpack_level(i, N, K, plans, ws, idx, dmin, st);
        if (filter && dmin && dmin[i]) {
            const PreparedView pv = prepared_view(prepared[i], C[i], K[i]);
            launch_exact_dist(x[i], x_bf16, pv.E4, plans[i].Kp, pv.enorm, idx[i], N[i], C[i], dmin[i], st);
        }
    }
    return hipGetLastError();
}

hipError_t launch_assign(const void* x, int x_bf16, int64_t N, int C, int K, const void* prepared, const VqPlan& p, char* ws,
                         int64_t* idx, float* dmin, hipStream_t st, const float* codebook) {
    return launch_assign_group(1, &x, x_bf16, &N, &C, &K, &prepared, &p, &ws, &idx, &dmin, p.T, st, codebook ? &codebook : nullptr);
}

KmPlan km_plan(int64_t N, int C, int K) {
    KmPlan p;
    p.vq = vq_plan(N, C, K);
    size_t off = p.vq.bytes;
    p.off_idx = off;
    off += (size_t)N * sizeof(int64_t);
    p.off_counts = off;
    off += (size_t)round_up(K + 1, 64) * sizeof(int);
    p.off_offsets = off;
    off += (size_t)round_up(K + 1, 64) * sizeof(int);
    p.off_members = off;
    off += (size_t)N * sizeof(int);
    p.off_sums = off;
    off += (size_t)K * C * sizeof(float);
    p.off_counts64 = off;
    off += (size_t)round_up(K, 32) * sizeof(int64_t);
    p.row_blocks = (int)((N + KM_RB - 1) / KM_RB);
    p.max_segments = (int)(N / KM_SEG + K);
    p.off_hist = off;
    off += (size_t)round_up(p.row_blocks * K, 64) * sizeof(int);
    p.off_segoff = off;
    off += (size_t)round_up(K + 1, 64) * sizeof(int);
    p.off_partial = off;
    off += (size_t)p.max_segments * C * sizeof(float);
    p.bytes = up256(off);
    return p;
}

hipError_t launch_km_accumulate(const float* samples, const float* means, int64_t N, int C, int K, const KmPlan& p,
                                char* ws, float* sums, int64_t* counts64, hipStream_t st) {
    hipError_t e = launch_prepare(means, K, C, ws + p.vq.off_prepared, st);
    if (e != hipSuccess) return e;
    int64_t* idx = reinterpret_cast<int64_t*>(ws + p.off_idx);
    e = launch_assign(samples, 0, N, C, K, ws + p.vq.off_prepared, p.vq, ws, idx, nullptr, st);
    if (e != hipSuccess) return e;
    return launch_code_sums(samples, 0, idx, N, C, K, p, ws, sums, counts64, st);
}

}
```

vq_seg_amd/csrc/vq_internal.h:

```cpp
#pragma once
#include "nn_device.h"
#include "vq_kernels.h"

namespace vqseg {

typedef float f32x16 __attribute__((ext_vector_type(16)));
typedef float f32x4 __attribute__((ext_vector_type(4)));
typedef unsigned int u32x2 __attribute__((ext_vector_type(2)));
typedef unsigned int u32x4 __attribute__((ext_vector_type(4)));

constexpr int ROWS_PER_WG = 128;
constexpr int F_ROWS = 128, F_CODES = 256, F_SUB = 128;
constexpr int F_LISTS = 64;
constexpr int GATHER_BLOCKS_MAX = 2048;
constexpr int GATHER_ROWS_PER_BLOCK = 16;
constexpr int KM_RB = 1024;
constexpr int KM_SEG = 128;

constexpr int VQ_ROWS_F32 = 0, VQ_ROWS_BF16 = 1, VQ_ROWS_S3 = 2;
__device__ __forceinline__ float s3_elem(const unsigned short* row, int C, int c) {
    return __builtin_bit_cast(float, (unsigned)row[c] << 16) + __builtin_bit_cast(float, (unsigned)row[C + c] << 16);
}

struct VqLevel {
    const void* x;
    const float* E4;
    const float* enorm;
    unsigned long long* keys;
    long N;
    int C, Kp;
    unsigned wg_end;
    const int* gate = nullptr;
    int gate_cap = 0;
    int K = 0;
};
struct VqFilterLevel {
    const void* x;
    const unsigned short* Eb;
    const float* enorm;
    const float* en_max;
    unsigned long long* summary;
    float* brow;
    unsigned long long* pair_rc;
    int* pair_count;
    int pair_cap;
    unsigned long long* keys;
    const float* W;
    const float* E4;
    long N;
    int C, Kp;
    unsigned wg_end;
    unsigned rblk_end;
    unsigned sblk_end;
};
struct VqFilterGroup {
    VqFilterLevel lv[VQ_MAX_LEVELS];
    int n;
};
struct VqInitLevel {
    unsigned long long* keys;
    long n;
    int* amb;
    int* hist;
    int kp;
    unsigned end;
};
struct VqInitGroup {
    VqInitLevel lv[VQ_MAX_LEVELS];
    int n;
};

struct PreparedView {
    float* E4;
    float* enorm;
    float* en_max;
    unsigned short* Eb;
};
PreparedView prepared_view(const void* prepared, int C, int K);

void launch_assign_levels(const VqLevel* lv, int n, int T, int row_type, hipStream_t st);
void launch_prepare_filter(const float* W, int K, int C, int Kp, const float* enorm, unsigned short* Eb, float* en_max, hipStream_t st);
void launch_filter(const VqFilterGroup& fg, int row_type, int force_all, hipStream_t st);
void launch_exact_dist(const void* x, int row_type, const float* E4, int Kp, const float* enorm, const int64_t* idx, int64_t N, int C, float* dmin,
                       hipStream_t st);
void launch_group_init(const VqInitGroup& ig, hipStream_t st);
void launch_unpack_level(int i, const int64_t* N, const int* K, const VqPlan* plans, char* const* ws, int64_t* const* idx,
                         float* const* dmin, hipStream_t st);
void launch_prepare_exact(const float* W, int K, int C, int Kp, float* E4, float* enorm, hipStream_t st);

}
```

vq_seg_amd/csrc/vq_kernels.h:

```cpp
#pragma once
#include <hip/hip_runtime.h>
#include <stddef.h>
#include <stdint.h>

namespace vqseg {

constexpr int VQ_MAX_LEVELS = 4;

struct VqPlan {
    int Cp, Kp;
    int T;
    size_t off_prepared, off_keys, off_hist, off_partial, bytes;
    int gather_blocks;
    size_t off_summary, off_brow, off_amb, off_pair_rc;
    int pair_cap;
};
struct PreparedLayout {
    size_t off_e4, off_enorm, off_enmax, off_eb, bytes;
};
PreparedLayout prepared_layout(int C, int K);
int vq_set_option(const char* key, int value);
struct KmPlan {
    VqPlan vq;
    size_t off_idx, off_counts, off_offsets, off_members, off_sums, off_counts64, off_hist, off_segoff, off_partial, bytes;
    int row_blocks, max_segments;
};

hipError_t profile_begin(int capacity);
void profile_release();
int profile_collect(int max_records, int64_t* n, int* c, int* k, float* ms, int* kind);

VqPlan vq_plan(int64_t N, int C, int K);
KmPlan km_plan(int64_t N, int C, int K);

size_t prepared_bytes(int C, int K);
hipError_t launch_prepare(const float* W, int K, int C, void* prepared, hipStream_t st);
hipError_t launch_assign(const void* x, int x_bf16, int64_t N, int C, int K, const void* prepared, const VqPlan& p, char* ws,
                         int64_t* idx, float* dmin, hipStream_t st, const float* codebook = nullptr);
int vq_group_tiles(int n, const int64_t* N, const int* K);
hipError_t launch_assign_group(int n, const void* const* x, int x_bf16, const int64_t* N, const int* C, const int* K,
                               const void* const* prepared, const VqPlan* plans, char* const* ws, int64_t* const* idx,
                               float* const* dmin, int T, hipStream_t st, const float* const* codebooks = nullptr);
hipError_t launch_gather(const void* x, int bf16, const float* W, const int64_t* idx, int64_t N, int C, int K, int training,
                         float cw, const VqPlan& p, char* ws, void* quant, float* loss, float* dead, hipStream_t st);
hipError_t launch_backward(const float* gq, const float* gloss, const float* x, const float* q, int64_t N, int C,
                           float cw, float* gx, hipStream_t st);
hipError_t launch_backward_idx(const void* gq, const float* gloss, const void* x, const int64_t* idx, const float* W, int64_t N,
                               int C, float cw, void* gx, hipStream_t st);
hipError_t launch_km_accumulate(const float* samples, const float* means, int64_t N, int C, int K, const KmPlan& p,
                                char* ws, float* sums, int64_t* counts64, hipStream_t st);
hipError_t launch_code_sums(const void* x, int x_bf16, const int64_t* idx, int64_t N, int C, int K, const KmPlan& p, char* ws,
                            float* sums, int64_t* counts64, hipStream_t st);
hipError_t launch_ema_update(float* cluster_size, float* embed_avg, float* codebook, const float* sums, const int64_t* counts64,
                             int K, int C, float decay, float eps, float* total, hipStream_t st);
hipError_t launch_revive_candidates(const void* x, int x_bf16, int64_t N, int C, int K, uint64_t seed, const int64_t* t, int rank,
                                    int world, float* cand, float* ok, hipStream_t st);
hipError_t launch_ema_update_revive(float* cluster_size, float* embed_avg, float* codebook, const float* sums, const int64_t* counts64,
                                    int K, int C, float decay, float eps, float* scratch, const float* cand, const float* ok,
                                    float threshold, int64_t* t, int64_t* revived, hipStream_t st);
hipError_t launch_km_finalize(const float* sums, const int64_t* counts64, float* means, int C, int K, hipStream_t st);

}
```

vq_seg_amd/csrc/vq_tail.hip:

```cpp
#include <hip/hip_runtime.h>
#include <stdint.h>

#include "vq_internal.h"

namespace vqseg {

static_assert(F_LISTS + 1 <= 128, "the init launch zeroes 128 ints of a level's counter block");
__global__ __launch_bounds__(256) void vq_group_init_kernel(const VqInitGroup g) {
    int q = 0;
    while (q + 1 < g.n && blockIdx.x >= g.lv[q].end) ++q;
    const VqInitLevel& L = g.lv[q];
    const unsigned first = q ? g.lv[q - 1].end : 0u, nb = L.end - first, b = blockIdx.x - first;
    for (long i = (long)b * 256 + threadIdx.x; i < L.n; i += (long)nb * 256) L.keys[i] = ~0ull;
    if (b == 0) {
        if (L.amb && threadIdx.x < 128) L.amb[threadIdx.x] = 0;
        for (int k = threadIdx.x; k < L.kp; k += 256) L.hist[k] = 0;
    }
}

__global__ __launch_bounds__(256) void vq_unpack_keys(const unsigned long long* __restrict__ keys, long N,
                                                      long long* __restrict__ idx, float* __restrict__ dmin,
                                                      int* __restrict__ hist, int K, int lds_hist) {
    extern __shared__ int lh[];
    if (hist && lds_hist)
        for (int k = threadIdx.x; k < K; k += 256) lh[k] = 0;
    __syncthreads();
    for (long i = (long)blockIdx.x * 256 + threadIdx.x; i < N; i += (long)gridDim.x * 256) {
        const unsigned long long k = keys[i];
        unsigned code = (unsigned)(k & 0xffffffffull);
        if (code >= (unsigned)K) code = 0u;
        idx[i] = (long long)code;
        if (dmin) dmin[i] = __uint_as_float((unsigned int)(k >> 32));
        if (hist && code < (unsigned)K) atomicAdd((lds_hist ? lh : hist) + code, 1);
    }
    if (hist && lds_hist) {
        __syncthreads();
        for (int k = threadIdx.x; k < K; k += 256) {
            const int c = lh[k];
            if (c) atomicAdd(hist + k, c);
        }
    }
}

template <typename TA>
__device__ __forceinline__ f32x4 ld4(const TA* p, long v) {
    if constexpr (sizeof(TA) == 4) {
        return reinterpret_cast<const f32x4*>(p)[v];
    } else {
        const u32x2 r = reinterpret_cast<const u32x2*>(p)[v];
        return f32x4{__builtin_bit_cast(float, r[0] << 16), __builtin_bit_cast(float, r[0] & 0xFFFF0000u),
                     __builtin_bit_cast(float, r[1] << 16), __builtin_bit_cast(float, r[1] & 0xFFFF0000u)};
    }
}
template <typename TA>
__device__ __forceinline__ void st4(TA* p, long v, const f32x4& q) {
    if constexpr (sizeof(TA) == 4) {
        reinterpret_cast<f32x4*>(p)[v] = q;
    } else {
        u32x2 r;
#pragma unroll
        for (int e = 0; e < 2; ++e) {
            const __bf16 lo = (__bf16)q[2 * e], hi = (__bf16)q[2 * e + 1];
            r[e] = (unsigned)__builtin_bit_cast(unsigned short, lo) | ((unsigned)__builtin_bit_cast(unsigned short, hi) << 16);
        }
        reinterpret_cast<u32x2*>(p)[v] = r;
    }
}

template <typename TA>
__global__ __launch_bounds__(256) void vq_gather_kernel(const TA* __restrict__ x, const float* __restrict__ W,
                                                        const long long* __restrict__ idx, long N, int C,
                                                        int training, TA* __restrict__ quant,
                                                        float* __restrict__ partial) {
    const int lane = threadIdx.x & 63, wave = threadIdx.x >> 6;
    const int c4 = C >> 2;
    float sq = 0.0f;
    constexpr int RG = 4;
    for (long row0 = ((long)blockIdx.x * 4 + wave) * RG; row0 < N; row0 += (long)gridDim.x * 4 * RG) {
        long long k[RG];
#pragma unroll
        for (int j = 0; j < RG; ++j) k[j] = row0 + j < N ? idx[row0 + j] : 0;
        if constexpr (__is_same(TA, S3Row)) {
            for (int v = lane; v < (C >> 3); v += 64) {
                f32x4 e0[RG], e1[RG];
#pragma unroll
                for (int j = 0; j < RG; ++j)
                    if (row0 + j < N) {
                        e0[j] = reinterpret_cast<const f32x4*>(W + k[j] * (long)C)[2 * v];
                        e1[j] = reinterpret_cast<const f32x4*>(W + k[j] * (long)C)[2 * v + 1];
                    }
#pragma unroll
                for (int j = 0; j < RG; ++j)
                    if (row0 + j < N) {
                        const float q[8] = {e0[j][0], e0[j][1], e0[j][2], e0[j][3], e1[j][0], e1[j][1], e1[j][2], e1[j][3]};
                        s3_store8(reinterpret_cast<unsigned short*>(quant) + (row0 + j) * 2L * C, C, 8 * v, q);
                    }
            }
            continue;
        }
        for (int v = lane; v < c4; v += 64) {
            f32x4 e[RG], xv[RG];
#pragma unroll
            for (int j = 0; j < RG; ++j) {
                if (row0 + j < N) {
                    e[j] = reinterpret_cast<const f32x4*>(W + k[j] * (long)C)[v];
                    if (training) xv[j] = ld4<TA>(x + (row0 + j) * (long)C, v);
                }
            }
#pragma unroll
            for (int j = 0; j < RG; ++j) {
                if (row0 + j < N) {
                    TA* qr = quant + (row0 + j) * (long)C;
                    if (training) {
                        f32x4 q;
#pragma unroll
                        for (int i = 0; i < 4; ++i) {
                            q[i] = xv[j][i] + (e[j][i] - xv[j][i]);
                            const float dlt = q[i] - xv[j][i];
                            sq = __builtin_fmaf(dlt, dlt, sq);
                        }
                        st4<TA>(qr, v, q);
                    } else {
                        st4<TA>(qr, v, e[j]);
                    }
                }
            }
        }
    }
#pragma unroll
    for (int m = 32; m >= 1; m >>= 1) sq += __shfl_xor(sq, m);
    __shared__ float wsum[4];
    if (lane == 0) wsum[wave] = sq;
    __syncthreads();
    if (threadIdx.x == 0) partial[blockIdx.x] = (wsum[0] + wsum[1]) + (wsum[2] + wsum[3]);
}

__global__ __launch_bounds__(256) void vq_finalize_kernel(const float* __restrict__ partial, int n_partial,
                                                          const int* __restrict__ hist, int K, int training,
                                                          float commitment_weight, double numel,
                                                          float* __restrict__ loss, float* __restrict__ dead_pct) {
    __shared__ double sd[256];
    __shared__ int sz[256];
    double s = 0.0;
    for (int i = threadIdx.x; i < n_partial; i += 256) s += (double)partial[i];
    int z = 0;
    for (int k = threadIdx.x; k < K; k += 256) z += (hist[k] == 0);
    sd[threadIdx.x] = s;
    sz[threadIdx.x] = z;
    __syncthreads();
    for (int m = 128; m >= 1; m >>= 1) {
        if (threadIdx.x < m) {
            sd[threadIdx.x] += sd[threadIdx.x + m];
            sz[threadIdx.x] += sz[threadIdx.x + m];
        }
        __syncthreads();
    }
    if (threadIdx.x == 0) {
        float l = 0.0f;
        if (training && commitment_weight > 0.0f) l = (float)(sd[0] / numel) * commitment_weight;
        loss[0] = l;
        dead_pct[0] = 100.0f * ((float)sz[0] / (float)K);
    }
}

__global__ __launch_bounds__(256) void vq_backward_kernel(const float* __restrict__ gq, const float* __restrict__ gloss,
                                                          const float* __restrict__ x, const float* __restrict__ q,
                                                          long n4, float coef, float* __restrict__ gx) {
    const float k = gloss ? gloss[0] * coef : 0.0f;
    for (long i = (long)blockIdx.x * 256 + threadIdx.x; i < n4; i += (long)gridDim.x * 256) {
        const f32x4 g = reinterpret_cast<const f32x4*>(gq)[i];
        const f32x4 xv = reinterpret_cast<const f32x4*>(x)[i];
        const f32x4 qv = reinterpret_cast<const f32x4*>(q)[i];
        f32x4 o;
#pragma unroll
        for (int j = 0; j < 4; ++j) o[j] = __builtin_fmaf(k, xv[j] - qv[j], g[j]);
        reinterpret_cast<f32x4*>(gx)[i] = o;
    }
}

__global__ __launch_bounds__(256) void vq_backward_idx_kernel(const __bf16* __restrict__ gq, const float* __restrict__ gloss,
                                                              const __bf16* __restrict__ x, const long long* __restrict__ idx,
                                                              const float* __restrict__ W, long N, int C, float coef,
                                                              __bf16* __restrict__ gx) {
    const float k = gloss ? gloss[0] * coef : 0.0f;
    const int c4 = C >> 2;
    const long n4 = N * c4;
    for (long i = (long)blockIdx.x * 256 + threadIdx.x; i < n4; i += (long)gridDim.x * 256) {
        const long row = i / c4;
        const int v = (int)(i - row * c4);
        const f32x4 g = ld4<__bf16>(gq, i), xv = ld4<__bf16>(x, i);
        const f32x4 e = reinterpret_cast<const f32x4*>(W + idx[row] * (long)C)[v];
        f32x4 o;
#pragma unroll
        for (int j = 0; j < 4; ++j) o[j] = __builtin_fmaf(k, xv[j] - e[j], g[j]);
        st4<__bf16>(gx, i, o);
    }
}

void launch_group_init(const VqInitGroup& ig, hipStream_t st) {
    hipLaunchKernelGGL(vq_group_init_kernel, dim3(ig.lv[ig.n - 1].end), dim3(256), 0, st, ig);
}

void launch_unpack_level(int i, const int64_t* N, const int* K, const VqPlan* plans, char* const* ws, int64_t* const* idx,
                         float* const* dmin, hipStream_t st) {
    int* hist = reinterpret_cast<int*>(ws[i] + plans[i].off_hist);
    long blocks = (N[i] + 1023) / 1024;
    if (blocks > 512) blocks = 512;
    if (blocks < 1) blocks = 1;
    const int lds_hist = K[i] <= 8192;
    hipLaunchKernelGGL(vq_unpack_keys, dim3((unsigned)blocks), dim3(256), lds_hist ? (size_t)K[i] * sizeof(int) : 0, st,
                       reinterpret_cast<unsigned long long*>(ws[i] + plans[i].off_keys), (long)N[i],
                       reinterpret_cast<long long*>(idx[i]), dmin ? dmin[i] : nullptr, hist, K[i], lds_hist);
}

hipError_t launch_gather(const void* x, int bf16, const float* W, const int64_t* idx, int64_t N, int C, int K, int training,
                         float cw, const VqPlan& p, char* ws, void* quant, float* loss, float* dead, hipStream_t st) {
    int* hist = reinterpret_cast<int*>(ws + p.off_hist);
    float* partial = reinterpret_cast<float*>(ws + p.off_partial);
    if (bf16 == VQ_ROWS_S3)
        hipLaunchKernelGGL(vq_gather_kernel<S3Row>, dim3(p.gather_blocks), dim3(256), 0, st, static_cast<const S3Row*>(x), W,
                           reinterpret_cast<const long long*>(idx), (long)N, C, 0, static_cast<S3Row*>(quant), partial);
    else if (bf16)
        hipLaunchKernelGGL(vq_gather_kernel<__bf16>, dim3(p.gather_blocks), dim3(256), 0, st, static_cast<const __bf16*>(x), W,
                           reinterpret_cast<const long long*>(idx), (long)N, C, training, static_cast<__bf16*>(quant), partial);
    else
        hipLaunchKernelGGL(vq_gather_kernel<float>, dim3(p.gather_blocks), dim3(256), 0, st, static_cast<const float*>(x), W,
                           reinterpret_cast<const long long*>(idx), (long)N, C, training, static_cast<float*>(quant), partial);
    hipLaunchKernelGGL(vq_finalize_kernel, dim3(1), dim3(256), 0, st, partial, p.gather_blocks, hist, K, training, cw,
                       (double)N * (double)C, loss, dead);
    return hipGetLastError();
}

hipError_t launch_backward(const float* gq, const float* gloss, const float* x, const float* q, int64_t N, int C,
                           float cw, float* gx, hipStream_t st) {
    const long n4 = (long)N * C / 4;
    const float coef = (float)((double)cw * 2.0 / ((double)N * (double)C));
    long blocks = (n4 + 255) / 256;
    if (blocks > 4096) blocks = 4096;
    if (blocks < 1) blocks = 1;
    hipLaunchKernelGGL(vq_backward_kernel, dim3((unsigned)blocks), dim3(256), 0, st, gq, gloss, x, q, n4, coef, gx);
    return hipGetLastError();
}

hipError_t launch_backward_idx(const void* gq, const float* gloss, const void* x, const int64_t* idx, const float* W, int64_t N,
                               int C, float cw, void* gx, hipStream_t st) {
    const long n4 = (long)N * C / 4;
    const float coef = (float)((double)cw * 2.0 / ((double)N * (double)C));
    long blocks = (n4 + 255) / 256;
    if (blocks > 4096) blocks = 4096;
    if (blocks < 1) blocks = 1;
    hipLaunchKernelGGL(vq_backward_idx_kernel, dim3((unsigned)blocks), dim3(256), 0, st, static_cast<const __bf16*>(gq), gloss,
                       static_cast<const __bf16*>(x), reinterpret_cast<const long long*>(idx), W, (long)N, C, coef,
                       static_cast<__bf16*>(gx));
    return hipGetLastError();
}

}
```

vq_seg_amd/csrc/vqseg_abi.hip:

```cpp
#include <hip/hip_runtime.h>
#include <stdarg.h>
#include <stdio.h>
#include <string.h>

#include "../../include/vqseg.h"
#include "vq_kernels.h"

namespace {
thread_local char g_err[512] = "";

int fail(int code, const char* fmt, ...) {
    va_list ap;
    va_start(ap, fmt);
    vsnprintf(g_err, sizeof(g_err), fmt, ap);
    va_end(ap);
    return code;
}
int hip_fail(hipError_t e, const char* where) {
    snprintf(g_err, sizeof(g_err), "%s: %s", where, hipGetErrorString(e));
    return (int)e;
}
bool aligned16(const void* p) { return (reinterpret_cast<uintptr_t>(p) & 15u) == 0; }

int check_shape(int64_t n, int c, int k) {
    if (n <= 0 || c <= 0 || k <= 0) return fail(VQSEG_EINVAL, "n_rows, channels and n_codes must be positive (got %lld, %d, %d)", (long long)n, c, k);
    if (c % 4) return fail(VQSEG_EINVAL, "channels must be a multiple of 4 (got %d)", c);
    if (n > (int64_t)1 << 31) return fail(VQSEG_EINVAL, "n_rows too large (%lld)", (long long)n);
    return 0;
}
}

extern "C" {

int vqseg_set_error(int code, const char* msg) {
    snprintf(g_err, sizeof(g_err), "%s", msg);
    return code;
}

int vqseg_abi_version(void) { return VQSEG_ABI_VERSION; }
const char* vqseg_last_error(void) { return g_err; }

const char* vqseg_kernel_name(const char* entry) {
    if (!entry) return "";
    if (!strcmp(entry, "vqseg_vq_forward_f32") || !strcmp(entry, "vqseg_vq_assign_f32") ||
        !strcmp(entry, "vqseg_kmeans_f32") || !strcmp(entry, "vqseg_kmeans_accumulate_f32"))
        return "vq_assign_f32_kernel";
    if (!strcmp(entry, "vqseg_vq_backward_f32")) return "vq_backward_kernel";
    if (!strcmp(entry, "vqseg_kmeans_finalize_f32")) return "km_finalize_kernel";
    return "";
}

int vqseg_profile_begin(int capacity) {
    if (capacity <= 0 || capacity > (1 << 20)) return fail(VQSEG_EINVAL, "capacity out of range");
    hipError_t e = vqseg::profile_begin(capacity);
    if (e != hipSuccess) return hip_fail(e, "profile_begin");
    return 0;
}

int vqseg_profile_collect(int max_records, int64_t* n_rows_host, int* channels_host, int* n_codes_host, float* ms_host, int* kind_host) {
    if (max_records <= 0 || !n_rows_host || !channels_host || !n_codes_host || !ms_host)
        return fail(VQSEG_EINVAL, "bad argument");
    return vqseg::profile_collect(max_records, n_rows_host, channels_host, n_codes_host, ms_host, kind_host);
}

size_t vqseg_vq_workspace_bytes(int64_t n, int c, int k) {
    if (n <= 0 || c <= 0 || k <= 0) return 0;
    return vqseg::vq_plan(n, c, k).bytes;
}

size_t vqseg_vq_filter_counter_offset(int64_t n, int c, int k) {
    if (n <= 0 || c <= 0 || k <= 0) return 0;
    const vqseg::VqPlan p = vqseg::vq_plan(n, c, k);
    return p.off_amb == p.off_summary ? 0 : p.off_amb;
}

int vqseg_vq_tiles_per_wave(int n_levels, const int64_t* n_rows_host, const int* n_codes_host) {
    if (n_levels < 1 || n_levels > vqseg::VQ_MAX_LEVELS || !n_rows_host || !n_codes_host) return fail(VQSEG_EINVAL, "tiles_per_wave: bad argument");
    for (int i = 0; i < n_levels; ++i)
        if (n_rows_host[i] <= 0 || n_codes_host[i] <= 0) return fail(VQSEG_EINVAL, "tiles_per_wave: non-positive size");
    return vqseg::vq_group_tiles(n_levels, n_rows_host, n_codes_host);
}

size_t vqseg_vq_prepared_bytes(int c, int k) {
    if (c <= 0 || k <= 0) return 0;
    return vqseg::prepared_bytes(c, k);
}

int vqseg_vq_prepare_f32(const float* codebook, int c, int k, void* prepared, size_t prepared_bytes, void* stream) {
    if (int rc = check_shape(1, c, k)) return rc;
    if (!codebook || !prepared) return fail(VQSEG_EINVAL, "null pointer argument");
    if (!aligned16(codebook) || !aligned16(prepared)) return fail(VQSEG_EINVAL, "codebook and prepared must be 16-byte aligned");
    if (prepared_bytes < vqseg::prepared_bytes(c, k))
        return fail(VQSEG_ENOSPC, "prepared buffer %zu < %zu bytes", prepared_bytes, vqseg::prepared_bytes(c, k));
    hipError_t e = vqseg::launch_prepare(codebook, k, c, prepared, static_cast<hipStream_t>(stream));
    if (e != hipSuccess) return hip_fail(e, "vq codebook prepare");
    return 0;
}

static int vq_assign_any(const void* x, int x_bf16, const float* codebook, const void* prepared, int64_t n, int c, int k,
                         int64_t* idx, float* dmin, void* ws, size_t ws_bytes, void* stream) {
    if (int rc = check_shape(n, c, k)) return rc;
    if (x_bf16 && c % 8) return fail(VQSEG_EINVAL, "%s rows need channels %% 8 == 0", x_bf16 == 2 ? "split-3" : "bf16");
    if (!x || !idx || !ws || (!codebook && !prepared)) return fail(VQSEG_EINVAL, "null pointer argument");
    if (!aligned16(x) || !aligned16(ws) || !aligned16(prepared) || !aligned16(codebook))
        return fail(VQSEG_EINVAL, "x, codebook, prepared and workspace must be 16-byte aligned");
    const vqseg::VqPlan p = vqseg::vq_plan(n, c, k);
    if (ws_bytes < p.bytes) return fail(VQSEG_ENOSPC, "workspace %zu < %zu bytes", ws_bytes, p.bytes);
    hipStream_t st = static_cast<hipStream_t>(stream);
    char* w = static_cast<char*>(ws);
    if (!prepared) {
        hipError_t e = vqseg::launch_prepare(codebook, k, c, w + p.off_prepared, st);
        if (e != hipSuccess) return hip_fail(e, "vq codebook prepare");
        prepared = w + p.off_prepared;
    }
    hipError_t e = vqseg::launch_assign(x, x_bf16, n, c, k, prepared, p, w, idx, dmin, st, codebook);
    if (e != hipSuccess) return hip_fail(e, "vq_assign_f32_kernel");
    return 0;
}

int vqseg_vq_assign_f32(const float* x, const float* codebook, const void* prepared, int64_t n, int c, int k,
                        int64_t* idx, float* dmin, void* ws, size_t ws_bytes, void* stream) {
    return vq_assign_any(x, 0, codebook, prepared, n, c, k, idx, dmin, ws, ws_bytes, stream);
}

int vqseg_vq_assign_bf16(const void* x, const float* codebook, const void* prepared, int64_t n, int c, int k,
                         int64_t* idx, float* dmin, void* ws, size_t ws_bytes, void* stream) {
    return vq_assign_any(x, 1, codebook, prepared, n, c, k, idx, dmin, ws, ws_bytes, stream);
}

int vqseg_vq_assign_s3(const void* x, const float* codebook, const void* prepared, int64_t n, int c, int k,
                       int64_t* idx, float* dmin, void* ws, size_t ws_bytes, void* stream) {
    return vq_assign_any(x, 2, codebook, prepared, n, c, k, idx, dmin, ws, ws_bytes, stream);
}

static int vq_forward_any(const void* x, int bf16, const float* codebook, const void* prepared, int64_t n, int c, int k,
                          int training, float cw, void* quant, int64_t* idx, float* loss, float* dead_pct, float* dmin,
                          void* ws, size_t ws_bytes, void* stream) {
    if (!quant || !loss || !dead_pct || !codebook) return fail(VQSEG_EINVAL, "null pointer argument");
    if (!aligned16(quant)) return fail(VQSEG_EINVAL, "quant must be 16-byte aligned");
    if (int rc = vq_assign_any(x, bf16, codebook, prepared, n, c, k, idx, dmin, ws, ws_bytes, stream)) return rc;
    const vqseg::VqPlan p = vqseg::vq_plan(n, c, k);
    hipError_t e = vqseg::launch_gather(x, bf16, codebook, idx, n, c, k, training, cw, p, static_cast<char*>(ws), quant, loss,
                                        dead_pct, static_cast<hipStream_t>(stream));
    if (e != hipSuccess) return hip_fail(e, "vq_gather_kernel");
    return 0;
}

int vqseg_vq_forward_f32(const float* x, const float* codebook, const void* prepared, int64_t n, int c, int k,
                         int training, float cw, float* quant, int64_t* idx, float* loss, float* dead_pct, float* dmin,
                         void* ws, size_t ws_bytes, void* stream) {
    return vq_forward_any(x, 0, codebook, prepared, n, c, k, training, cw, quant, idx, loss, dead_pct, dmin, ws, ws_bytes, stream);
}

int vqseg_vq_forward_bf16(const void* x, const float* codebook, const void* prepared, int64_t n, int c, int k,
                          int training, float cw, void* quant, int64_t* idx, float* loss, float* dead_pct, float* dmin,
                          void* ws, size_t ws_bytes, void* stream) {
    return vq_forward_any(x, 1, codebook, prepared, n, c, k, training, cw, quant, idx, loss, dead_pct, dmin, ws, ws_bytes, stream);
}

int vqseg_vq_forward_group(int n_levels, int bf16, const void* const* x, const float* const* codebook, const void* const* prepared,
                           const int64_t* n, const int* c, const int* k, int training, const float* cw, void* const* quant,
                           int64_t* const* idx, float* const* loss, float* const* dead_pct, void* const* ws, const size_t* ws_bytes,
                           void* stream) {
    if (n_levels < 1 || n_levels > vqseg::VQ_MAX_LEVELS) return fail(VQSEG_EINVAL, "1 .. %d levels per grouped launch", vqseg::VQ_MAX_LEVELS);
    if (bf16 < 0 || bf16 > 2) return fail(VQSEG_EINVAL, "row type must be 0 (f32), 1 (bf16) or 2 (split-3), got %d", bf16);
    if (bf16 == 2 && training) return fail(VQSEG_EINVAL, "split-3 rows are an eval-mode format: training must be 0");
    if (!x || !codebook || !n || !c || !k || !cw || !quant || !idx || !loss || !dead_pct || !ws || !ws_bytes)
        return fail(VQSEG_EINVAL, "null pointer argument");
    vqseg::VqPlan plans[vqseg::VQ_MAX_LEVELS];
    const void* prep[vqseg::VQ_MAX_LEVELS];
    char* wsp[vqseg::VQ_MAX_LEVELS];
    hipStream_t st = static_cast<hipStream_t>(stream);
    for (int i = 0; i < n_levels; ++i) {
        if (int rc = check_shape(n[i], c[i], k[i])) return rc;
        if (bf16 && c[i] % 8) return fail(VQSEG_EINVAL, "%s rows need channels %% 8 == 0", bf16 == 2 ? "split-3" : "bf16");
        if (!x[i] || !codebook[i] || !quant[i] || !idx[i] || !loss[i] || !dead_pct[i] || !ws[i]) return fail(VQSEG_EINVAL, "null pointer argument");
        if (!aligned16(x[i]) || !aligned16(ws[i]) || !aligned16(codebook[i]) || !aligned16(quant[i]) || (prepared && !aligned16(prepared[i])))
            return fail(VQSEG_EINVAL, "x, codebook, prepared, quant and workspace must be 16-byte aligned");
        plans[i] = vqseg::vq_plan(n[i], c[i], k[i]);
        if (ws_bytes[i] < plans[i].bytes) return fail(VQSEG_ENOSPC, "workspace %zu < %zu bytes", ws_bytes[i], plans[i].bytes);
        wsp[i] = static_cast<char*>(ws[i]);
        prep[i] = prepared ? prepared[i] : nullptr;
        if (!prep[i]) {
            hipError_t e = vqseg::launch_prepare(codebook[i], k[i], c[i], wsp[i] + plans[i].off_prepared, st);
            if (e != hipSuccess) return hip_fail(e, "vq codebook prepare");
            prep[i] = wsp[i] + plans[i].off_prepared;
        }
    }
    const int T = vqseg::vq_group_tiles(n_levels, n, k);
    hipError_t e = vqseg::launch_assign_group(n_levels, x, bf16, n, c, k, prep, plans, wsp, idx, nullptr, T, st, codebook);
    if (e != hipSuccess) return hip_fail(e, "vq_assign_f32_kernel (grouped)");
    for (int i = 0; i < n_levels; ++i) {
        e = vqseg::launch_gather(x[i], bf16, codebook[i], idx[i], n[i], c[i], k[i], training, cw[i], plans[i], wsp[i], quant[i], loss[i],
                                 dead_pct[i], st);
        if (e != hipSuccess) return hip_fail(e, "vq_gather_kernel");
    }
    return 0;
}

int vqseg_vq_backward_bf16(const void* gq, const float* gloss, const void* x, const int64_t* idx, const float* codebook,
                           int64_t n, int c, float cw, void* gx, void* stream) {
    if (int rc = check_shape(n, c, 1)) return rc;
    if (!gq || !x || !idx || !codebook || !gx) return fail(VQSEG_EINVAL, "null pointer argument");
    if (c % 8) return fail(VQSEG_EINVAL, "bf16 rows need channels %% 8 == 0");
    if (!aligned16(gq) || !aligned16(x) || !aligned16(codebook) || !aligned16(gx)) return fail(VQSEG_EINVAL, "tensors must be 16-byte aligned");
    hipError_t e = vqseg::launch_backward_idx(gq, gloss, x, idx, codebook, n, c, cw, gx, static_cast<hipStream_t>(stream));
    if (e != hipSuccess) return hip_fail(e, "vq_backward_idx_kernel");
    return 0;
}

int vqseg_vq_backward_f32(const float* gq, const float* gloss, const float* x, const float* quant, int64_t n, int c,
                          float cw, float* gx, void* stream) {
    if (int rc = check_shape(n, c, 1)) return rc;
    if (!gq || !x || !quant || !gx) return fail(VQSEG_EINVAL, "null pointer argument");
    if (!aligned16(gq) || !aligned16(x) || !aligned16(quant) || !aligned16(gx))
        return fail(VQSEG_EINVAL, "tensors must be 16-byte aligned");
    hipError_t e = vqseg::launch_backward(gq, gloss, x, quant, n, c, cw, gx, static_cast<hipStream_t>(stream));
    if (e != hipSuccess) return hip_fail(e, "vq_backward_kernel");
    return 0;
}

size_t vqseg_kmeans_workspace_bytes(int64_t n, int c, int k) {
    if (n <= 0 || c <= 0 || k <= 0) return 0;
    return vqseg::km_plan(n, c, k).bytes;
}

int vqseg_kmeans_accumulate_f32(const float* samples, const float* means, int64_t n, int c, int k, float* sums,
                                int64_t* counts, void* ws, size_t ws_bytes, void* stream) {
    if (int rc = check_shape(n, c, k)) return rc;
    if (!samples || !means || !sums || !counts || !ws) return fail(VQSEG_EINVAL, "null pointer argument");
    if (!aligned16(samples) || !aligned16(ws)) return fail(VQSEG_EINVAL, "samples and workspace must be 16-byte aligned");
    const vqseg::KmPlan p = vqseg::km_plan(n, c, k);
    if (ws_bytes < p.bytes) return fail(VQSEG_ENOSPC, "workspace %zu < %zu bytes", ws_bytes, p.bytes);
    hipError_t e = vqseg::launch_km_accumulate(samples, means, n, c, k, p, static_cast<char*>(ws), sums, counts,
                                               static_cast<hipStream_t>(stream));
    if (e != hipSuccess) return hip_fail(e, "kmeans accumulate");
    return 0;
}

int vqseg_vq_code_sums(int bf16, const void* x, const int64_t* idx, int64_t n, int c, int k, float* sums, int64_t* counts, void* ws,
                       size_t ws_bytes, void* stream) {
    if (int rc = check_shape(n, c, k)) return rc;
    if (!x || !idx || !sums || !counts || !ws) return fail(VQSEG_EINVAL, "null pointer argument");
    if (!aligned16(ws)) return fail(VQSEG_EINVAL, "workspace must be 16-byte aligned");
    const vqseg::KmPlan p = vqseg::km_plan(n, c, k);
    if (ws_bytes < p.bytes) return fail(VQSEG_ENOSPC, "workspace %zu < %zu bytes", ws_bytes, p.bytes);
    hipError_t e = vqseg::launch_code_sums(x, bf16 != 0, idx, n, c, k, p, static_cast<char*>(ws), sums, counts,
                                           static_cast<hipStream_t>(stream));
    if (e != hipSuccess) return hip_fail(e, "code sums");
    return 0;
}

int vqseg_vq_ema_update_f32(float* cluster_size, float* embed_avg, float* codebook, const float* sums, const int64_t* counts, int c,
                            int k, float decay, float eps, float* scratch, void* stream) {
    if (c <= 0 || k <= 0 || !cluster_size || !embed_avg || !codebook || !sums || !counts || !scratch)
        return fail(VQSEG_EINVAL, "bad argument");
    if (!(decay >= 0.0f && decay <= 1.0f) || !(eps >= 0.0f)) return fail(VQSEG_EINVAL, "need 0 <= decay <= 1, eps >= 0");
    hipError_t e = vqseg::launch_ema_update(cluster_size, embed_avg, codebook, sums, counts, k, c, decay, eps, scratch,
                                            static_cast<hipStream_t>(stream));
    if (e != hipSuccess) return hip_fail(e, "ema_embed_kernel");
    return 0;
}

int vqseg_vq_revive_candidates(int bf16, const void* x, int64_t n, int c, int k, uint64_t seed, const int64_t* counter, int rank,
                               int world, float* cand, float* ok, void* stream) {
    if (!x || !counter || !cand || !ok) return fail(VQSEG_EINVAL, "revive candidates: null pointer argument");
    if (n < 1 || k < 1) return fail(VQSEG_EINVAL, "revive candidates: n_rows and n_codes must be positive (got %lld, %d)", (long long)n, k);
    if (n > (int64_t)1 << 31) return fail(VQSEG_EINVAL, "n_rows too large (%lld)", (long long)n);
    if (world < 1) return fail(VQSEG_EINVAL, "revive candidates: world must be >= 1 (got %d)", world);
    if (rank < 0 || rank >= world) return fail(VQSEG_EINVAL, "revive candidates: rank %d outside [0, %d)", rank, world);
    if (c <= 0 || c % 4) return fail(VQSEG_EINVAL, "channels must be a multiple of 4 (got %d)", c);
    if (bf16 && c % 8) return fail(VQSEG_EINVAL, "bf16 rows need channels %% 8 == 0");
    if (!aligned16(x) || !aligned16(cand)) return fail(VQSEG_EINVAL, "rows and cand must be 16-byte aligned");
    hipError_t e = vqseg::launch_revive_candidates(x, bf16 != 0, n, c, k, seed, counter, rank, world, cand, ok,
                                                   static_cast<hipStream_t>(stream));
    if (e != hipSuccess) return hip_fail(e, "revive_candidates_kernel");
    return 0;
}

int vqseg_vq_ema_update_revive_f32(float* cluster_size, float* embed_avg, float* codebook, const float* sums, const int64_t* counts,
                                   int c, int k, float decay, float eps, float* scratch, const float* cand, const float* ok,
                                   float threshold, int64_t* counter, int64_t* revived, void* stream) {
    if (c <= 0 || k <= 0 || !cluster_size || !embed_avg || !codebook || !sums || !counts || !scratch)
        return fail(VQSEG_EINVAL, "bad argument");
    if (!cand || !ok || !counter || !revived) return fail(VQSEG_EINVAL, "ema update with revival: null pointer argument");
    if (!(decay >= 0.0f && decay <= 1.0f) || !(eps >= 0.0f)) return fail(VQSEG_EINVAL, "need 0 <= decay <= 1, eps >= 0");
    if (!(threshold >= 0.0f) || threshold > 3.0e38f) return fail(VQSEG_EINVAL, "need a finite threshold >= 0");
    hipError_t e = vqseg::launch_ema_update_revive(cluster_size, embed_avg, codebook, sums, counts, k, c, decay, eps, scratch, cand, ok,
                                                   threshold, counter, revived, static_cast<hipStream_t>(stream));
    if (e != hipSuccess) return hip_fail(e, "ema_embed_revive_kernel");
    return 0;
}

int vqseg_kmeans_finalize_f32(const float* sums, const int64_t* counts, float* means, int c, int k, void* stream) {
    if (c <= 0 || k <= 0 || !sums || !counts || !means) return fail(VQSEG_EINVAL, "bad argument");
    hipError_t e = vqseg::launch_km_finalize(sums, counts, means, c, k, static_cast<hipStream_t>(stream));
    if (e != hipSuccess) return hip_fail(e, "km_finalize_kernel");
    return 0;
}

int vqseg_kmeans_f32(const float* samples, float* means, int64_t* bins, int64_t n, int c, int k, int iters, void* ws,
                     size_t ws_bytes, void* stream) {
    if (int rc = check_shape(n, c, k)) return rc;
    if (!samples || !means || !bins || !ws) return fail(VQSEG_EINVAL, "null pointer argument");
    if (iters < 0) return fail(VQSEG_EINVAL, "iters must be >= 0");
    const vqseg::KmPlan p = vqseg::km_plan(n, c, k);
    if (ws_bytes < p.bytes) return fail(VQSEG_ENOSPC, "workspace %zu < %zu bytes", ws_bytes, p.bytes);
    char* w = static_cast<char*>(ws);
    float* sums = reinterpret_cast<float*>(w + p.off_sums);
    hipStream_t st = static_cast<hipStream_t>(stream);
    for (int it = 0; it < iters; ++it) {
        if (int rc = vqseg_kmeans_accumulate_f32(samples, means, n, c, k, sums, bins, ws, ws_bytes, stream)) return rc;
        hipError_t e = vqseg::launch_km_finalize(sums, bins, means, c, k, st);
        if (e != hipSuccess) return hip_fail(e, "km_finalize_kernel");
    }
    return 0;
}

}
```

vq_seg_amd/models/networks/modified_vqunet/net.py:

```python
import torch
from torch import nn

from .... import nnf
from ....vector_quantizer import make_vq_module, Identity as _IdentityVQ, quantize_group as _quantize_group
from ...encoders import make_encoder
from ...modules.prototype import ReliablePrototypeLoss, ReliablePrototypeLossv2
from ..unet.decoder import UnetDecoder
from ..unet.net import _to_device_layout


class _Upsampling(nn.Module):

    def __init__(self, scale_factor):
        super().__init__()
        self.scale_factor = scale_factor

    def forward(self, x):
        return nnf.upsample_bilinear(x, scale_factor=self.scale_factor, align_corners=True)


class _Head1x1(nn.Conv2d):
    def forward(self, x):
        return nnf.head_conv1x1(x, self.weight)


class _VQRePTUnet1x1Base(nn.Module):
    _proto_cls = None

    def __init__(self, encoder_name: str, num_classes: int, vq_cfg: dict, margin=1.5, scale=1., use_feature=False,
                 encoder_weights=None, in_channels: int = 3, decoder_channels=None, depth: int = 5,
                 activation=nn.Identity, upsampling=2, pt_init="kmeans"):
        super().__init__()
        self.encoder = make_encoder(encoder_name, in_channels, depth, weights=encoder_weights, padding_mode="reflect")
        enc_ch = self.encoder.out_channels()
        self.codebook = make_vq_module(vq_cfg, enc_ch, depth)
        if decoder_channels is None:
            decoder_channels = [c // 2 for c in enc_ch[1:]][::-1]
        self.decoder = UnetDecoder(enc_ch, decoder_channels)
        self.segmentation_head = _Head1x1(decoder_channels[-1], num_classes, 1, bias=False)
        self.prototype_loss = self._proto_cls(num_classes, decoder_channels[-1], margin=margin, scale=scale, init=pt_init,
                                              use_feature=use_feature)
        self.device = None
        self.upsampling = _Upsampling(upsampling) if upsampling > 1 else nn.Identity()

    def encode(self, x):
        if self.device is None:
            self.device = x.device
        with nnf.s3_scope(not self.training and not torch.is_grad_enabled()):
            feats = self.encoder(_to_device_layout(x))[1:]
        if len(feats) != len(self.codebook):
            raise NotImplementedError
        return feats

    def quantize(self, feats):
        loss = torch.zeros(1, device=feats[0].device)
        usage = []
        levels = [i for i, vq in enumerate(self.codebook) if not isinstance(vq, _IdentityVQ)]
        vqs = [self.codebook[i] for i in levels]
        group = nnf.py_opt("py_vq_group", 1)
        grouped = None
        if group and nnf.py_opt("py_vq_s3", 1) and any(isinstance(feats[i], nnf.S3) for i in levels):
            grouped = _quantize_group(vqs, [feats[i] for i in levels])
        if grouped is None:
            for i in levels:
                if isinstance(feats[i], nnf.S3):
                    feats[i] = feats[i].float()
            grouped = _quantize_group(vqs, [feats[i] for i in levels]) if group else None
        grouped = dict(zip(levels, grouped)) if grouped is not None else {}
        for i, vq in enumerate(self.codebook):
            quantize, _idx, commitment, dead = grouped[i] if i in grouped else vq(feats[i])
            feats[i] = quantize
            if commitment is not None:
                loss = loss + commitment
            if dead is not None:
                usage.append(dead.detach())
        return feats, loss / len(feats), usage

    def decode(self, feats):
        decoder_out = self.decoder(*feats)
        if self.training:
            nnf.fanin_tag(decoder_out)
        return decoder_out, self.segmentation_head(decoder_out)

    def _side_terms(self, decoder_out, gt, side):
        if side is None or not self.training:
            return
        if side.get("sup_con") is not None:
            side["sup_con_loss"] = side["sup_con"](decoder_out, gt)
        if side.get("keep"):
            side["decoder_out"] = decoder_out.detach()

    def _trunk(self, x):
        feats, loss, usage = self.quantize(self.encode(x))
        decoder_out, logits = self.decode(feats)
        return decoder_out, logits, loss, usage

    async_code_usage = False

    def _usage_to_host(self, usage, like):
        if not usage:
            return torch.tensor([])
        stacked = torch.stack(usage)
        if not (self.async_code_usage and stacked.is_cuda):
            return stacked.cpu()
        ring = self.__dict__.setdefault("_usage_ring", [])
        if len(ring) < 8:
            ring.append(torch.empty(stacked.shape, dtype=stacked.dtype, pin_memory=True))
        buf = ring[self.__dict__.setdefault("_usage_i", 0) % len(ring)]
        self.__dict__["_usage_i"] += 1
        buf.copy_(stacked, non_blocking=True)
        return buf

    @torch.no_grad()
    def pseudo_label(self, x):
        _, logits, _, _ = self._trunk(x)
        return torch.argmax(logits, dim=1).long()


class VQRePTUnet1x1(_VQRePTUnet1x1Base):
    _proto_cls = ReliablePrototypeLoss

    def forward(self, x, gt=None, code_usage_loss=False, percent=None):
        return self.finish(*self.quantize(self.encode(x)), gt=gt, code_usage_loss=code_usage_loss, percent=percent)

    def finish(self, feats, loss, usage, gt=None, code_usage_loss=False, percent=None, side=None):
        decoder_out, output = self.decode(feats)
        self._side_terms(decoder_out, gt, side)
        prototype_loss = None
        if self.training:
            with torch.no_grad():
                if nnf.softmax_stats_supported(output):
                    entropy = nnf.softmax_stats(output, want_label=False)[1].reshape(-1)
                else:
                    prob = torch.softmax(output.float().permute(0, 2, 3, 1).reshape(-1, output.shape[1]), dim=1)
                    entropy = -torch.sum(prob * torch.log(prob + 1e-10), dim=1)
            prototype_loss = self.prototype_loss(decoder_out, gt, percent=percent, entropy=entropy)
        output = self.upsampling(output)
        if code_usage_loss:
            return output, loss, self._usage_to_host(usage, output), torch.stack(usage).sum()[None] / len(self.codebook)
        return output, loss, self._usage_to_host(usage, output), prototype_loss


class VQRePTUnet1x1v2(_VQRePTUnet1x1Base):
    _proto_cls = ReliablePrototypeLossv2

    def forward(self, x, gt=None, code_usage_loss=False, th=None):
        return self.finish(*self.quantize(self.encode(x)), gt=gt, code_usage_loss=code_usage_loss, th=th)

    def finish(self, feats, loss, usage, gt=None, code_usage_loss=False, th=None, side=None):
        decoder_out, output = self.decode(feats)
        self._side_terms(decoder_out, gt, side)
        prototype_loss = self.prototype_loss(decoder_out, gt, th) if self.training else None
        output = self.upsampling(output)
        if code_usage_loss:
            return output, loss, self._usage_to_host(usage, output), torch.stack(usage).sum()[None] / len(self.codebook)
        return output, loss, self._usage_to_host(usage, output), prototype_loss
```

vq_seg_amd/vector_quantizer/vq_img.py:

```python
from __future__ import annotations

import torch
from torch import nn

from .. import _hip
from .. import nnf
from .._wcache import cache_of as _cache_of, invalidate as _invalidate
from ..dist import collectives_on as _collectives_on, broadcast0 as _broadcast0, all_reduce_sum as _all_reduce_sum, rank as _rank, \
    world_size as _world_size


class _VQFunction(torch.autograd.Function):

    @staticmethod
    def forward(ctx, rows, codebook, training, commitment_weight, prepared=None):
        quant, idx, loss, dead = _hip.vq_forward(rows, codebook, training, commitment_weight, prepared=prepared)
        ctx.commitment_weight = float(commitment_weight)
        ctx.training = bool(training)
        ctx.bf16 = rows.dtype == torch.bfloat16
        if training:
            if ctx.bf16:
                ctx.save_for_backward(rows, idx, codebook)
            else:
                ctx.save_for_backward(rows, quant)
        ctx.mark_non_differentiable(idx, dead)
        return quant, idx, loss, dead

    @staticmethod
    def backward(ctx, g_quant, _g_idx, g_loss, _g_dead):
        if not ctx.training:
            return None, None, None, None, None
        gl = g_loss.contiguous() if (g_loss is not None and ctx.commitment_weight > 0) else None
        if ctx.bf16:
            rows, idx, codebook = ctx.saved_tensors
            g_quant = torch.zeros_like(rows) if g_quant is None else g_quant.to(torch.bfloat16).contiguous()
            return _hip.vq_backward_bf16(g_quant, gl, rows, idx, codebook, ctx.commitment_weight), None, None, None, None
        rows, quant = ctx.saved_tensors
        if g_quant is None:
            g_quant = torch.zeros_like(rows)
        g_quant = g_quant.contiguous()
        gx = _hip.vq_backward(g_quant, gl, rows, quant, ctx.commitment_weight)
        return gx, None, None, None, None


class _VQGroupFunction(torch.autograd.Function):

    @staticmethod
    def forward(ctx, training, weights, n, fans, *tensors):
        rows, codebooks, prepared = tensors[:n], tensors[n:2 * n], tensors[2 * n:3 * n]
        ctx.fans = fans
        outs = _hip.vq_forward_group(list(rows), list(codebooks), list(prepared), training, weights)
        ctx.n, ctx.training, ctx.weights = n, bool(training), [float(w) for w in weights]
        ctx.bf16 = rows[0].dtype == torch.bfloat16
        if training:
            saved = []
            for r, cb, (q, idx, _l, _d) in zip(rows, codebooks, outs):
                saved += [r, idx, cb] if ctx.bf16 else [r, q]
            ctx.save_for_backward(*saved)
        flat, nondiff = [], []
        for q, idx, loss, dead in outs:
            nondiff += [idx, dead]
            flat += [q, idx, loss, dead]
        ctx.mark_non_differentiable(*nondiff)
        return tuple(flat)

    @staticmethod
    def backward(ctx, *grads):
        n = ctx.n
        none = (None, None, None, None) + (None,) * (3 * n)
        if not ctx.training:
            return none
        saved = ctx.saved_tensors
        gxs = []
        for i in range(n):
            g_quant, g_loss = grads[4 * i], grads[4 * i + 2]
            w = ctx.weights[i]
            gl = g_loss.contiguous() if (g_loss is not None and w > 0) else None
            if ctx.bf16:
                rows, idx, codebook = saved[3 * i:3 * i + 3]
                g_quant = torch.zeros_like(rows) if g_quant is None else g_quant.to(torch.bfloat16).contiguous()
                gxs.append(_hip.vq_backward_bf16(g_quant, gl, rows, idx, codebook, w))
            else:
                rows, quant = saved[2 * i:2 * i + 2]
                g_quant = torch.zeros_like(rows) if g_quant is None else g_quant.contiguous()
                gxs.append(_hip.vq_backward(g_quant, gl, rows, quant, w))
            fan = ctx.fans[i] if ctx.fans is not None else None
            if fan is not None and gxs[-1].dtype == fan[2] and nnf._fanin_deposit(fan[0], gxs[-1].reshape(fan[1])):
                gxs[-1] = None
        return (None, None, None, None) + tuple(gxs) + (None,) * (2 * n)


def quantize_group(vqs, feats):
    if len(vqs) < 2 or len(vqs) > 4:
        return None
    if any(isinstance(f, nnf.S3) for f in feats):
        return _quantize_group_s3(vqs, feats)
    rows = []
    for vq, f in zip(vqs, feats):
        cb = vq.codebook
        if not torch.is_tensor(f) or not f.is_cuda or cb.ema_update or (cb.kmeans_init and vq.training and not cb.initted):
            return None
        rows.append(_rows_of(f))
    if len({r.dtype for r in rows}) != 1 or len({vq.training for vq in vqs}) != 1:
        return None
    n = len(vqs)
    weights = [float(vq.commitment_weight) for vq in vqs]
    fans = None
    if vqs[0].training and torch.is_grad_enabled():
        fans = []
        for f, r in zip(feats, rows):
            link = nnf._fanin_of(f)
            b, c, h, w = f.shape
            fans.append((link, (b, h, w, c), f.dtype) if (link is not None and r.dtype == f.dtype and r.data_ptr() == f.data_ptr()) else None)
        if not any(fans):
            fans = None
    flat = _VQGroupFunction.apply(vqs[0].training, weights, n, fans, *rows, *[vq.codebook.embedding.weight.detach() for vq in vqs],
                                  *[vq.codebook.prepared() for vq in vqs])
    outs = []
    for i, f in enumerate(feats):
        b, c, h, w = f.shape
        quant, idx, loss, dead = flat[4 * i:4 * i + 4]
        outs.append((quant.reshape(b, h, w, c).permute(0, 3, 1, 2), idx.reshape(b, h, w), loss, dead))
    return outs


def _quantize_group_s3(vqs, feats):
    if not all(isinstance(f, nnf.S3) for f in feats) or torch.is_grad_enabled():
        return None
    L = _hip.lib()
    for vq, f in zip(vqs, feats):
        cb = vq.codebook
        b, c, h, w = f.shape
        if vq.training or cb.ema_update or not f.rows.is_cuda or c != cb.embedding_dim or \
                not L.vqseg_vq_filter_counter_offset(b * h * w, c, cb.num_embeddings):
            return None
    rows = [f.rows.reshape(-1, 2 * f.c) for f in feats]
    res = _hip.vq_forward_group(rows, [vq.codebook.embedding.weight.detach() for vq in vqs], [vq.codebook.prepared() for vq in vqs],
                                False, [float(vq.commitment_weight) for vq in vqs], s3=True)
    outs = []
    for f, (quant, idx, loss, dead) in zip(feats, res):
        b, c, h, w = f.shape
        outs.append((nnf.s3_from_rows(quant.reshape(b, h, w, 2 * c), c), idx.reshape(b, h, w), loss, dead))
    return outs


def _rows_of(x: torch.Tensor):
    b, c, h, w = x.shape
    if not (x.dtype == torch.bfloat16 and x.is_cuda and c % 8 == 0 and torch.is_autocast_enabled()):
        x = x.to(torch.float32)
    rows = x.permute(0, 2, 3, 1)
    if not rows.is_contiguous():
        rows = rows.contiguous()
    return rows.reshape(b * h * w, c)


def kmeans_init_means(rows: torch.Tensor, num_clusters: int) -> torch.Tensor:
    n = rows.shape[0]
    if n >= num_clusters:
        pick = torch.randperm(n, device=rows.device)[:num_clusters]
    else:
        pick = torch.randint(0, n, (num_clusters,), device=rows.device)
    return rows[pick].contiguous()


def kmeans(rows: torch.Tensor, num_clusters: int, num_iters: int, init_means: torch.Tensor = None):
    means = (kmeans_init_means(rows, num_clusters) if init_means is None else init_means.clone()).contiguous()
    if not _collectives_on():
        return _hip.kmeans(rows, means, num_iters)
    _broadcast0(means)
    counts = torch.zeros(num_clusters, dtype=torch.int64, device=rows.device)
    for _ in range(num_iters):
        sums, counts = _hip.kmeans_accumulate(rows, means)
        _all_reduce_sum(sums)
        _all_reduce_sum(counts)
        _hip.kmeans_finalize(sums, counts, means)
    return means, counts


class EuclideanCodebook(nn.Module):
    def __init__(self, embedding_dim, num_embeddings, kmeans_init, kmeans_iters, decay, eps, num_codebook, ema_update=False,
                 threshold_ema_dead_code: float = 0.0, revive_seed: int = 0):
        super().__init__()
        if threshold_ema_dead_code < 0:
            raise ValueError(f"threshold_ema_dead_code must be >= 0, got {threshold_ema_dead_code}")
        if threshold_ema_dead_code > 0 and not ema_update:
            raise ValueError("threshold_ema_dead_code > 0 revives codes of the EMA update: it needs ema_update=True")
        self.kmeans_init = kmeans_init
        self.kmeans_iters = kmeans_iters
        self.initted = False
        self.num_codebook = num_codebook
        self.decay = decay
        self.eps = eps
        self.ema_update = bool(ema_update)
        self.embedding = nn.Embedding(num_embeddings, embedding_dim)
        self.num_embeddings = num_embeddings
        self.embedding_dim = embedding_dim
        if not kmeans_init:
            self.embedding.weight.data.uniform_(-1 / num_embeddings, 1 / num_embeddings)
            self.initted = True
        if self.ema_update:
            self.register_buffer("cluster_size", torch.zeros(num_embeddings))
            self.register_buffer("embed_avg", self.embedding.weight.detach().clone())
        self.threshold_ema_dead_code = float(threshold_ema_dead_code)
        self.revive_seed = int(revive_seed)
        self.revived = None
        if self.threshold_ema_dead_code > 0:
            self.register_buffer("ema_updates", torch.zeros((), dtype=torch.int64))

    def prepared(self) -> torch.Tensor:
        w = self.embedding.weight
        cache = _cache_of(w)
        if "vq_prepared" not in cache:
            cache["vq_prepared"] = _hip.vq_prepare(w.detach())
        return cache["vq_prepared"]

    @torch.no_grad()
    def _kmeans_init(self, rows: torch.Tensor):
        if self.initted:
            return
        means, bins = kmeans(rows, self.num_embeddings, self.kmeans_iters)
        self.embedding.weight.copy_(means)
        _invalidate(self.embedding.weight)
        if self.ema_update:
            self.embed_avg.copy_(means)
            self.cluster_size.copy_(bins.to(self.cluster_size.dtype))
        self.initted = True

    @torch.no_grad()
    def ema_step(self, rows: torch.Tensor, idx: torch.Tensor):
        if self.threshold_ema_dead_code > 0:
            return self._ema_revive_step(rows, idx)
        sums, counts = _hip.vq_code_sums(rows, idx.reshape(-1), self.num_embeddings)
        if _collectives_on():
            _all_reduce_sum(sums)
            _all_reduce_sum(counts)
        _hip.vq_ema_update(self.cluster_size, self.embed_avg, self.embedding.weight.detach(), sums, counts, self.decay, self.eps)
        _invalidate(self.embedding.weight)

    def _ema_revive_step(self, rows: torch.Tensor, idx: torch.Tensor):
        k, c = self.num_embeddings, self.embedding_dim
        flat = torch.empty(2 * k * c + k, dtype=torch.float32, device=rows.device)
        sums, cand, ok = flat[:k * c].view(k, c), flat[k * c:2 * k * c].view(k, c), flat[2 * k * c:]
        _, counts = _hip.vq_code_sums(rows, idx.reshape(-1), k, out=sums)
        _hip.vq_revive_candidates(rows, self.revive_seed, self.ema_updates, k, _rank(), _world_size(), out=(cand, ok))
        if _collectives_on():
            _all_reduce_sum(flat)
            _all_reduce_sum(counts)
        if self.revived is None or self.revived.device != rows.device:
            self.revived = torch.zeros((), dtype=torch.int64, device=rows.device)
        _hip.vq_ema_update(self.cluster_size, self.embed_avg, self.embedding.weight.detach(), sums, counts, self.decay, self.eps,
                           candidates=cand, ok=ok, threshold=self.threshold_ema_dead_code, counter=self.ema_updates, revived=self.revived)
        _invalidate(self.embedding.weight)

    def forward(self, x: torch.Tensor):
        b, hw, c = x.shape
        rows = x.float().reshape(b * hw, c).contiguous()
        if self.kmeans_init and self.training:
            self._kmeans_init(rows.detach())
        quant, idx, _loss, dead = _VQFunction.apply(rows.detach(), self.embedding.weight.detach(), False, 0.0,
                                                    self.prepared())
        return quant.reshape(b, hw, c), idx.reshape(b, hw), dead


class VectorQuantizer(nn.Module):
    def __init__(self, dim, num_embeddings, embedding_dim=None, decay=0.8, eps=1e-5, kmeans_init=False,
                 kmeans_iters=10, distance="euclidean", commitment_weight=1, num_codebook=1, ema_update=False,
                 threshold_ema_dead_code: float = 0.0, revive_seed: int = 0):
        super().__init__()
        embedding_dim = embedding_dim if embedding_dim is not None else dim
        self.num_embeddings = num_embeddings
        self.eps = eps
        self.commitment_weight = commitment_weight
        if distance != "euclidean":
            raise NotImplementedError(
                f"distance={distance!r}: only the euclidean codebook is on the accelerated path (SURVEY 2 #1; the "
                "cosine codebook is unused by the target configs)")
        self.codebook = EuclideanCodebook(embedding_dim=embedding_dim, num_embeddings=num_embeddings,
                                          kmeans_init=kmeans_init, kmeans_iters=kmeans_iters, decay=decay, eps=eps,
                                          num_codebook=num_codebook, ema_update=ema_update,
                                          threshold_ema_dead_code=threshold_ema_dead_code, revive_seed=revive_seed)

    def forward(self, x: torch.Tensor):
        b, c, h, w = x.shape
        rows = _rows_of(x)
        cb = self.codebook
        if cb.kmeans_init and self.training and not cb.initted:
            cb._kmeans_init(rows.detach().float())
        ema = cb.ema_update and self.training
        weight = cb.embedding.weight.detach()
        if ema:
            weight = weight.clone()
        quant, idx, loss, dead = _VQFunction.apply(rows, weight, self.training, float(self.commitment_weight), cb.prepared())
        if ema:
            cb.ema_step(rows.detach(), idx)
        quantize = quant.reshape(b, h, w, c).permute(0, 3, 1, 2)
        return quantize, idx.reshape(b, h, w), loss, dead
```

Before: 446.6 images/sec.

## Fuse grouped VQ unpack, gather and finalize into single tail launches with fused loss mean

Result: no change. 448.0 images/sec (median of 6 runs) (+0.3%).

```diff
diff --git a/include/vqseg.h b/include/vqseg.h
--- a/include/vqseg.h
+++ b/include/vqseg.h
@@ -41,6 +41,13 @@
                            int training, const float* commitment_weight, void* const* quant, int64_t* const* idx,
                            float* const* loss, float* const* dead_pct, void* const* workspace,
                            const size_t* workspace_bytes, void* stream);
+
+int vqseg_vq_forward_group_mean(int n_levels, int bf16, const void* const* x, const float* const* codebook,
+                                const void* const* prepared, const int64_t* n_rows, const int* channels, const int* n_codes,
+                                int training, const float* commitment_weight, void* const* quant, int64_t* const* idx,
+                                float* const* loss, float* const* dead_pct, int n_feats, float* mean, void* const* workspace,
+                                const size_t* workspace_bytes, void* stream);
+int vqseg_vq_group_tail(void);
 
 size_t vqseg_vq_filter_counter_offset(int64_t n_rows, int channels, int n_codes);
 
diff --git a/vq_seg_amd/_hip.py b/vq_seg_amd/_hip.py
--- a/vq_seg_amd/_hip.py
+++ b/vq_seg_amd/_hip.py
@@ -28,6 +28,9 @@
     "vqseg_vq_forward_bf16": (c_int, [c_void_p, c_void_p, c_void_p, c_int64, c_int, c_int, c_int, c_float, c_void_p,
                                       c_void_p, c_void_p, c_void_p, c_void_p, c_void_p, c_size_t, c_void_p]),
     "vqseg_vq_forward_group": (c_int, [c_int, c_int] + [c_void_p] * 6 + [c_int, c_void_p] + [c_void_p] * 6 + [c_void_p]),
+    "vqseg_vq_forward_group_mean": (c_int, [c_int, c_int] + [c_void_p] * 6 + [c_int, c_void_p] + [c_void_p] * 4 + [c_int, c_void_p] +
+                                    [c_void_p] * 2 + [c_void_p]),
+    "vqseg_vq_group_tail": (c_int, []),
     "vqseg_vq_backward_bf16": (c_int, [c_void_p, c_void_p, c_void_p, c_void_p, c_void_p, c_int64, c_int, c_float, c_void_p, c_void_p]),
     "vqseg_vq_assign_f32": (c_int, [c_void_p, c_void_p, c_void_p, c_int64, c_int, c_int, c_void_p, c_void_p, c_void_p,
                                     c_size_t, c_void_p]),
@@ -311,7 +314,12 @@
     return _bind_symbols(ctypes.CDLL(path))
 
 
-def vq_forward_group(rows_list, codebooks, prepared_list, training: bool, commitment_weights, handle=None, s3: bool = False):
+def vq_group_tail() -> bool:
+    return bool(lib().vqseg_vq_group_tail())
+
+
+def vq_forward_group(rows_list, codebooks, prepared_list, training: bool, commitment_weights, handle=None, s3: bool = False,
+                     n_feats: Optional[int] = None):
     L = handle or lib()
     nl = len(rows_list)
     bf16 = 2 if s3 else int(rows_list[0].dtype == torch.bfloat16)
@@ -338,15 +346,18 @@
     for w, p_ in zip(codebooks, prepared_list):
         preps.append(tptr(p_, "prepared codebook", dtype=torch.uint8, numel=L.vqseg_vq_prepared_bytes(w.shape[1], w.shape[0])))
     wsb = (c_size_t * nl)(*[w.numel() for w in wss])
-    launch("vqseg_vq_forward_group", dev, nl, bf16, ptr(xs), ptr(wps), ptr(preps), ns.ctypes.data, cs.ctypes.data, ks.ctypes.data,
+    mean = torch.empty(1, dtype=torch.float32, device=dev) if n_feats is not None else None
+    launch("vqseg_vq_forward_group" if mean is None else "vqseg_vq_forward_group_mean", dev, nl, bf16, ptr(xs), ptr(wps), ptr(preps),
+           ns.ctypes.data, cs.ctypes.data, ks.ctypes.data,
            int(bool(training)), cw.ctypes.data, ptr(q.data_ptr() for q in quants), ptr(i.data_ptr() for i in idxs),
-           ptr(s.data_ptr() for s in scals), ptr(s.data_ptr() + 4 for s in scals), ptr(w.data_ptr() for w in wss),
-           ctypes.cast(wsb, c_void_p), handle=handle)
+           ptr(s.data_ptr() for s in scals), ptr(s.data_ptr() + 4 for s in scals), *(() if mean is None else (int(n_feats), mean.data_ptr())),
+           ptr(w.data_ptr() for w in wss), ctypes.cast(wsb, c_void_p), handle=handle)
     if FILTER_DIAG is not None and bf16:
         for r, w, ws_ in zip(rows_list, codebooks, wss):
             off = L.vqseg_vq_filter_counter_offset(r.shape[0], w.shape[1], w.shape[0])
             FILTER_DIAG.append((r.shape[0], w.shape[1], w.shape[0], ws_[off:off + 256].view(torch.int32) if off else None))
-    return [(q, i, s[0:1], s[1]) for q, i, s in zip(quants, idxs, scals)]
+    outs = [(q, i, s[0:1], s[1]) for q, i, s in zip(quants, idxs, scals)]
+    return outs if mean is None else (outs, mean)
 
 
 def set_option(key: str, value: int) -> int:
diff --git a/vq_seg_amd/csrc/vq_host.hip b/vq_seg_amd/csrc/vq_host.hip
--- a/vq_seg_amd/csrc/vq_host.hip
+++ b/vq_seg_amd/csrc/vq_host.hip
@@ -40,6 +40,7 @@
 static int g_vq_filter_force_all = 0;
 static int g_vq_filter_launches = 0;
 static int g_vq_s3_filter = 1;
+static int g_vq_group_tail = 1;
 static const Option VQ_OPTIONS[] = {
     {"vq_max_tiles_per_wave", &g_vq_max_tiles, OPT_POW2_FAIL, 1, 8},
     {"vq_fine_split", &g_vq_fine_split, OPT_FLAG},
@@ -47,9 +48,11 @@
     {"vq_filter_force_all", &g_vq_filter_force_all, OPT_FLAG},
     {"vq_filter_launches", &g_vq_filter_launches},
     {"vq_s3_filter", &g_vq_s3_filter, OPT_FLAG},
+    {"vq_group_tail", &g_vq_group_tail, OPT_FLAG},
 };
 
 int vq_set_option(const char* key, int value) { return apply_option(VQ_OPTIONS, key, value); }
+bool vq_group_tail_on() { return g_vq_group_tail != 0; }
 
 VqPlan vq_plan(int64_t N, int C, int K) {
     VqPlan p;
@@ -180,9 +183,15 @@
     return 1;
 }
 
+static long unpack_blocks(int64_t N) {
+    long blocks = (N + 1023) / 1024;
+    if (blocks > 512) blocks = 512;
+    return blocks < 1 ? 1 : blocks;
+}
+
 hipError_t launch_assign_group(int n, const void* const* x, int x_bf16, const int64_t* N, const int* C, const int* K,
                                const void* const* prepared, const VqPlan* plans, char* const* ws, int64_t* const* idx,
-                               float* const* dmin, int T, hipStream_t st, const float* const* codebooks) {
+                               float* const* dmin, int T, hipStream_t st, const float* const* codebooks, bool unpack) {
     if (n < 1 || n > VQ_MAX_LEVELS) return hipErrorInvalidValue;
     int order[VQ_MAX_LEVELS];
     for (int i = 0; i < n; ++i) order[i] = i;
@@ -245,7 +254,7 @@
     launch_assign_levels(lv, n, T, x_bf16, st);
     if (rec) (void)hipEventRecord(g_prof.ev[2 * slot + 1], st);
     hipError_t e = hipGetLastError();
-    if (e != hipSuccess) return e;
+    if (e != hipSuccess || !unpack) return e;
     for (int i = 0; i < n; ++i) {
         launch_unpack_level(i, N, K, plans, ws, idx, dmin, st);
         if (filter && dmin && dmin[i]) {
@@ -253,6 +262,36 @@
             launch_exact_dist(x[i], x_bf16, pv.E4, plans[i].Kp, pv.enorm, idx[i], N[i], C[i], dmin[i], st);
         }
     }
+    return hipGetLastError();
+}
+
+hipError_t launch_group_forward_tail(int n, const void* const* x, int bf16, const float* const* W, const int64_t* N, const int* C,
+                                     const int* K, int training, const float* cw, const VqPlan* plans, char* const* ws,
+                                     int64_t* const* idx, void* const* quant, float* const* loss, float* const* dead, int n_feats,
+                                     float* mean, hipStream_t st) {
+    if (n < 1 || n > VQ_MAX_LEVELS) return hipErrorInvalidValue;
+    VqTailGroup tg;
+    VqFinalGroup fg;
+    tg.n = fg.n = n;
+    tg.training = fg.training = bf16 == VQ_ROWS_S3 ? 0 : training;
+    unsigned gend = 0, uend = 0;
+    size_t lds_bytes = 0;
+    for (int i = 0; i < n; ++i) {
+        int* hist = reinterpret_cast<int*>(ws[i] + plans[i].off_hist);
+        float* partial = reinterpret_cast<float*>(ws[i] + plans[i].off_partial);
+        const int lds_hist = K[i] <= 8192;
+        if (lds_hist && (size_t)K[i] * sizeof(int) > lds_bytes) lds_bytes = (size_t)K[i] * sizeof(int);
+        gend += (unsigned)plans[i].gather_blocks;
+        uend += (unsigned)unpack_blocks(N[i]);
+        tg.lv[i] = VqTailLevel{reinterpret_cast<const unsigned long long*>(ws[i] + plans[i].off_keys), reinterpret_cast<long long*>(idx[i]),
+                               hist, x[i], W[i], quant[i], partial, (long)N[i], C[i], K[i], lds_hist, gend, uend};
+        fg.lv[i] = VqFinalLevel{partial, hist, loss[i], dead[i], (double)N[i] * (double)C[i], plans[i].gather_blocks, K[i], cw[i]};
+    }
+    tg.n_gather = gend;
+    fg.inv_feats = n_feats > 0 ? 1.0f / (float)n_feats : 0.0f;
+    fg.mean = mean;
+    launch_group_tail(tg, bf16, lds_bytes, uend, st);
+    launch_group_finalize(fg, st);
     return hipGetLastError();
 }
 
diff --git a/vq_seg_amd/csrc/vq_internal.h b/vq_seg_amd/csrc/vq_internal.h
--- a/vq_seg_amd/csrc/vq_internal.h
+++ b/vq_seg_amd/csrc/vq_internal.h
@@ -70,6 +70,43 @@
     int n;
 };
 
+struct VqTailLevel {
+    const unsigned long long* keys;
+    long long* idx;
+    int* hist;
+    const void* x;
+    const float* W;
+    void* quant;
+    float* partial;
+    long N;
+    int C, K;
+    int lds_hist;
+    unsigned gather_end;
+    unsigned unpack_end;
+};
+struct VqTailGroup {
+    VqTailLevel lv[VQ_MAX_LEVELS];
+    int n;
+    unsigned n_gather;
+    int training;
+};
+struct VqFinalLevel {
+    const float* partial;
+    const int* hist;
+    float* loss;
+    float* dead_pct;
+    double numel;
+    int n_partial, K;
+    float cw;
+};
+struct VqFinalGroup {
+    VqFinalLevel lv[VQ_MAX_LEVELS];
+    int n;
+    int training;
+    float inv_feats;
+    float* mean;
+};
+
 struct PreparedView {
     float* E4;
     float* enorm;
@@ -86,6 +123,8 @@
 void launch_group_init(const VqInitGroup& ig, hipStream_t st);
 void launch_unpack_level(int i, const int64_t* N, const int* K, const VqPlan* plans, char* const* ws, int64_t* const* idx,
                          float* const* dmin, hipStream_t st);
+void launch_group_tail(const VqTailGroup& tg, int row_type, size_t lds_bytes, unsigned n_unpack, hipStream_t st);
+void launch_group_finalize(const VqFinalGroup& fg, hipStream_t st);
 void launch_prepare_exact(const float* W, int K, int C, int Kp, float* E4, float* enorm, hipStream_t st);
 
 }
diff --git a/vq_seg_amd/csrc/vq_kernels.h b/vq_seg_amd/csrc/vq_kernels.h
--- a/vq_seg_amd/csrc/vq_kernels.h
+++ b/vq_seg_amd/csrc/vq_kernels.h
@@ -40,7 +40,12 @@
 int vq_group_tiles(int n, const int64_t* N, const int* K);
 hipError_t launch_assign_group(int n, const void* const* x, int x_bf16, const int64_t* N, const int* C, const int* K,
                                const void* const* prepared, const VqPlan* plans, char* const* ws, int64_t* const* idx,
-                               float* const* dmin, int T, hipStream_t st, const float* const* codebooks = nullptr);
+                               float* const* dmin, int T, hipStream_t st, const float* const* codebooks = nullptr, bool unpack = true);
+bool vq_group_tail_on();
+hipError_t launch_group_forward_tail(int n, const void* const* x, int bf16, const float* const* W, const int64_t* N, const int* C,
+                                     const int* K, int training, const float* cw, const VqPlan* plans, char* const* ws,
+                                     int64_t* const* idx, void* const* quant, float* const* loss, float* const* dead, int n_feats,
+                                     float* mean, hipStream_t st);
 hipError_t launch_gather(const void* x, int bf16, const float* W, const int64_t* idx, int64_t N, int C, int K, int training,
                          float cw, const VqPlan& p, char* ws, void* quant, float* loss, float* dead, hipStream_t st);
 hipError_t launch_backward(const float* gq, const float* gloss, const float* x, const float* q, int64_t N, int C,
diff --git a/vq_seg_amd/csrc/vq_tail.hip b/vq_seg_amd/csrc/vq_tail.hip
--- a/vq_seg_amd/csrc/vq_tail.hip
+++ b/vq_seg_amd/csrc/vq_tail.hip
@@ -67,19 +67,17 @@
     }
 }
 
-template <typename TA>
-__global__ __launch_bounds__(256) void vq_gather_kernel(const TA* __restrict__ x, const float* __restrict__ W,
-                                                        const long long* __restrict__ idx, long N, int C,
-                                                        int training, TA* __restrict__ quant,
-                                                        float* __restrict__ partial) {
+template <typename TA, typename CodeOf>
+__device__ __forceinline__ float gather_rows(const TA* __restrict__ x, const float* __restrict__ W, CodeOf code_of, long N, int C,
+                                             int training, TA* __restrict__ quant, unsigned blk, unsigned nblk) {
     const int lane = threadIdx.x & 63, wave = threadIdx.x >> 6;
     const int c4 = C >> 2;
     float sq = 0.0f;
     constexpr int RG = 4;
-    for (long row0 = ((long)blockIdx.x * 4 + wave) * RG; row0 < N; row0 += (long)gridDim.x * 4 * RG) {
+    for (long row0 = ((long)blk * 4 + wave) * RG; row0 < N; row0 += (long)nblk * 4 * RG) {
         long long k[RG];
 #pragma unroll
-        for (int j = 0; j < RG; ++j) k[j] = row0 + j < N ? idx[row0 + j] : 0;
+        for (int j = 0; j < RG; ++j) k[j] = row0 + j < N ? code_of(row0 + j) : 0;
         if constexpr (__is_same(TA, S3Row)) {
             for (int v = lane; v < (C >> 3); v += 64) {
                 f32x4 e0[RG], e1[RG];
@@ -127,12 +125,70 @@
             }
         }
     }
+    return sq;
+}
+__device__ __forceinline__ void gather_fold(float sq, float* __restrict__ out) {
+    const int lane = threadIdx.x & 63, wave = threadIdx.x >> 6;
 #pragma unroll
     for (int m = 32; m >= 1; m >>= 1) sq += __shfl_xor(sq, m);
     __shared__ float wsum[4];
     if (lane == 0) wsum[wave] = sq;
     __syncthreads();
-    if (threadIdx.x == 0) partial[blockIdx.x] = (wsum[0] + wsum[1]) + (wsum[2] + wsum[3]);
+    if (threadIdx.x == 0) *out = (wsum[0] + wsum[1]) + (wsum[2] + wsum[3]);
+}
+
+template <typename TA>
+__global__ __launch_bounds__(256) void vq_gather_kernel(const TA* __restrict__ x, const float* __restrict__ W,
+                                                        const long long* __restrict__ idx, long N, int C,
+                                                        int training, TA* __restrict__ quant,
+                                                        float* __restrict__ partial) {
+    const float sq = gather_rows<TA>(x, W, [idx](long r) { return idx[r]; }, N, C, training, quant, blockIdx.x, gridDim.x);
+    gather_fold(sq, partial + blockIdx.x);
+}
+
+template <typename TA>
+__global__ __launch_bounds__(256) void vq_group_tail_kernel(const VqTailGroup g) {
+    extern __shared__ int lh[];
+    int q = 0;
+    if (blockIdx.x < g.n_gather) {
+        while (q + 1 < g.n && blockIdx.x >= g.lv[q].gather_end) ++q;
+        const VqTailLevel& L = g.lv[q];
+        const unsigned first = q ? g.lv[q - 1].gather_end : 0u;
+        const unsigned long long* __restrict__ keys = L.keys;
+        const unsigned K = (unsigned)L.K;
+        const float sq = gather_rows<TA>(static_cast<const TA*>(L.x), L.W,
+                                         [keys, K](long r) {
+                                             const unsigned code = (unsigned)(keys[r] & 0xffffffffull);
+                                             return (long long)(code >= K ? 0u : code);
+                                         },
+                                         L.N, L.C, g.training, static_cast<TA*>(L.quant), blockIdx.x - first, L.gather_end - first);
+        gather_fold(sq, L.partial + (blockIdx.x - first));
+        return;
+    }
+    const unsigned ub = blockIdx.x - g.n_gather;
+    while (q + 1 < g.n && ub >= g.lv[q].unpack_end) ++q;
+    const VqTailLevel& L = g.lv[q];
+    const unsigned first = q ? g.lv[q - 1].unpack_end : 0u, nb = L.unpack_end - first, b = ub - first;
+    const int K = L.K, lds_hist = L.lds_hist;
+    const unsigned long long* __restrict__ keys = L.keys;
+    long long* __restrict__ idx = L.idx;
+    int* __restrict__ hist = L.hist;
+    if (lds_hist)
+        for (int k = threadIdx.x; k < K; k += 256) lh[k] = 0;
+    __syncthreads();
+    for (long i = (long)b * 256 + threadIdx.x; i < L.N; i += (long)nb * 256) {
+        unsigned code = (unsigned)(keys[i] & 0xffffffffull);
+        if (code >= (unsigned)K) code = 0u;
+        idx[i] = (long long)code;
+        atomicAdd((lds_hist ? lh : hist) + code, 1);
+    }
+    if (lds_hist) {
+        __syncthreads();
+        for (int k = threadIdx.x; k < K; k += 256) {
+            const int c = lh[k];
+            if (c) atomicAdd(hist + k, c);
+        }
+    }
 }
 
 __global__ __launch_bounds__(256) void vq_finalize_kernel(const float* __restrict__ partial, int n_partial,
@@ -163,6 +219,38 @@
     }
 }
 
+__global__ __launch_bounds__(256) void vq_group_finalize_kernel(const VqFinalGroup g) {
+    __shared__ double sd[256];
+    __shared__ int sz[256];
+    float m = 0.0f;
+    for (int q = 0; q < g.n; ++q) {
+        const VqFinalLevel& L = g.lv[q];
+        double s = 0.0;
+        for (int i = threadIdx.x; i < L.n_partial; i += 256) s += (double)L.partial[i];
+        int z = 0;
+        for (int k = threadIdx.x; k < L.K; k += 256) z += (L.hist[k] == 0);
+        sd[threadIdx.x] = s;
+        sz[threadIdx.x] = z;
+        __syncthreads();
+        for (int w = 128; w >= 1; w >>= 1) {
+            if (threadIdx.x < w) {
+                sd[threadIdx.x] += sd[threadIdx.x + w];
+                sz[threadIdx.x] += sz[threadIdx.x + w];
+            }
+            __syncthreads();
+        }
+        if (threadIdx.x == 0) {
+            float l = 0.0f;
+            if (g.training && L.cw > 0.0f) l = __fmul_rn((float)(sd[0] / L.numel), L.cw);
+            L.loss[0] = l;
+            L.dead_pct[0] = 100.0f * ((float)sz[0] / (float)L.K);
+            m = __fadd_rn(m, l);
+        }
+        __syncthreads();
+    }
+    if (threadIdx.x == 0 && g.mean) g.mean[0] = __fmul_rn(m, g.inv_feats);
+}
+
 __global__ __launch_bounds__(256) void vq_backward_kernel(const float* __restrict__ gq, const float* __restrict__ gloss,
                                                           const float* __restrict__ x, const float* __restrict__ q,
                                                           long n4, float coef, float* __restrict__ gx) {
@@ -211,6 +299,26 @@
     hipLaunchKernelGGL(vq_unpack_keys, dim3((unsigned)blocks), dim3(256), lds_hist ? (size_t)K[i] * sizeof(int) : 0, st,
                        reinterpret_cast<unsigned long long*>(ws[i] + plans[i].off_keys), (long)N[i],
                        reinterpret_cast<long long*>(idx[i]), dmin ? dmin[i] : nullptr, hist, K[i], lds_hist);
+}
+
+void launch_group_tail(const VqTailGroup& tg, int row_type, size_t lds_bytes, unsigned n_unpack, hipStream_t st) {
+    auto launch = [&](const VqTailGroup& g, unsigned grid, size_t lds) {
+        if (row_type == VQ_ROWS_S3) hipLaunchKernelGGL(vq_group_tail_kernel<S3Row>, dim3(grid), dim3(256), lds, st, g);
+        else if (row_type == VQ_ROWS_BF16) hipLaunchKernelGGL(vq_group_tail_kernel<__bf16>, dim3(grid), dim3(256), lds, st, g);
+        else hipLaunchKernelGGL(vq_group_tail_kernel<float>, dim3(grid), dim3(256), lds, st, g);
+    };
+    if (lds_bytes <= 16384) {
+        launch(tg, tg.n_gather + n_unpack, lds_bytes);
+        return;
+    }
+    VqTailGroup ug = tg;
+    ug.n_gather = 0;
+    launch(ug, n_unpack, lds_bytes);
+    launch(tg, tg.n_gather, 0);
+}
+
+void launch_group_finalize(const VqFinalGroup& fg, hipStream_t st) {
+    hipLaunchKernelGGL(vq_group_finalize_kernel, dim3(1), dim3(256), 0, st, fg);
 }
 
 hipError_t launch_gather(const void* x, int bf16, const float* W, const int64_t* idx, int64_t N, int C, int K, int training,
diff --git a/vq_seg_amd/csrc/vqseg_abi.hip b/vq_seg_amd/csrc/vqseg_abi.hip
--- a/vq_seg_amd/csrc/vqseg_abi.hip
+++ b/vq_seg_amd/csrc/vqseg_abi.hip
@@ -158,10 +158,10 @@
     return vq_forward_any(x, 1, codebook, prepared, n, c, k, training, cw, quant, idx, loss, dead_pct, dmin, ws, ws_bytes, stream);
 }
 
-int vqseg_vq_forward_group(int n_levels, int bf16, const void* const* x, const float* const* codebook, const void* const* prepared,
-                           const int64_t* n, const int* c, const int* k, int training, const float* cw, void* const* quant,
-                           int64_t* const* idx, float* const* loss, float* const* dead_pct, void* const* ws, const size_t* ws_bytes,
-                           void* stream) {
+static int vq_forward_group_any(int n_levels, int bf16, const void* const* x, const float* const* codebook, const void* const* prepared,
+                                const int64_t* n, const int* c, const int* k, int training, const float* cw, void* const* quant,
+                                int64_t* const* idx, float* const* loss, float* const* dead_pct, int n_feats, float* mean,
+                                void* const* ws, const size_t* ws_bytes, void* stream) {
     if (n_levels < 1 || n_levels > vqseg::VQ_MAX_LEVELS) return fail(VQSEG_EINVAL, "1 .. %d levels per grouped launch", vqseg::VQ_MAX_LEVELS);
     if (bf16 < 0 || bf16 > 2) return fail(VQSEG_EINVAL, "row type must be 0 (f32), 1 (bf16) or 2 (split-3), got %d", bf16);
     if (bf16 == 2 && training) return fail(VQSEG_EINVAL, "split-3 rows are an eval-mode format: training must be 0");
@@ -188,8 +188,15 @@
         }
     }
     const int T = vqseg::vq_group_tiles(n_levels, n, k);
-    hipError_t e = vqseg::launch_assign_group(n_levels, x, bf16, n, c, k, prep, plans, wsp, idx, nullptr, T, st, codebook);
+    const bool group_tail = vqseg::vq_group_tail_on();
+    hipError_t e = vqseg::launch_assign_group(n_levels, x, bf16, n, c, k, prep, plans, wsp, idx, nullptr, T, st, codebook, !group_tail);
     if (e != hipSuccess) return hip_fail(e, "vq_assign_f32_kernel (grouped)");
+    if (group_tail) {
+        e = vqseg::launch_group_forward_tail(n_levels, x, bf16, codebook, n, c, k, training, cw, plans, wsp, idx, quant, loss, dead_pct,
+                                             n_feats, mean, st);
+        if (e != hipSuccess) return hip_fail(e, "vq_group_tail_kernel");
+        return 0;
+    }
     for (int i = 0; i < n_levels; ++i) {
         e = vqseg::launch_gather(x[i], bf16, codebook[i], idx[i], n[i], c[i], k[i], training, cw[i], plans[i], wsp[i], quant[i], loss[i],
                                  dead_pct[i], st);
@@ -197,6 +204,27 @@
     }
     return 0;
 }
+
+int vqseg_vq_forward_group(int n_levels, int bf16, const void* const* x, const float* const* codebook, const void* const* prepared,
+                           const int64_t* n, const int* c, const int* k, int training, const float* cw, void* const* quant,
+                           int64_t* const* idx, float* const* loss, float* const* dead_pct, void* const* ws, const size_t* ws_bytes,
+                           void* stream) {
+    return vq_forward_group_any(n_levels, bf16, x, codebook, prepared, n, c, k, training, cw, quant, idx, loss, dead_pct, 0, nullptr, ws,
+                                ws_bytes, stream);
+}
+
+int vqseg_vq_forward_group_mean(int n_levels, int bf16, const void* const* x, const float* const* codebook, const void* const* prepared,
+                                const int64_t* n, const int* c, const int* k, int training, const float* cw, void* const* quant,
+                                int64_t* const* idx, float* const* loss, float* const* dead_pct, int n_feats, float* mean,
+                                void* const* ws, const size_t* ws_bytes, void* stream) {
+    if (!mean) return fail(VQSEG_EINVAL, "null pointer argument");
+    if (n_feats < n_levels) return fail(VQSEG_EINVAL, "the mean runs over n_feats >= n_levels features (got %d for %d levels)", n_feats, n_levels);
+    if (!vqseg::vq_group_tail_on()) return fail(VQSEG_EINVAL, "the mean term is written by the grouped tail: option vq_group_tail is 0");
+    return vq_forward_group_any(n_levels, bf16, x, codebook, prepared, n, c, k, training, cw, quant, idx, loss, dead_pct, n_feats, mean, ws,
+                                ws_bytes, stream);
+}
+
+int vqseg_vq_group_tail(void) { return vqseg::vq_group_tail_on() ? 1 : 0; }
 
 int vqseg_vq_backward_bf16(const void* gq, const float* gloss, const void* x, const int64_t* idx, const float* codebook,
                            int64_t n, int c, float cw, void* gx, void* stream) {
diff --git a/vq_seg_amd/models/networks/modified_vqunet/net.py b/vq_seg_amd/models/networks/modified_vqunet/net.py
--- a/vq_seg_amd/models/networks/modified_vqunet/net.py
+++ b/vq_seg_amd/models/networks/modified_vqunet/net.py
@@ -34,6 +34,8 @@
         self.encoder = make_encoder(encoder_name, in_channels, depth, weights=encoder_weights, padding_mode="reflect")
         enc_ch = self.encoder.out_channels()
         self.codebook = make_vq_module(vq_cfg, enc_ch, depth)
+        for vq in self.codebook:
+            vq.loss_mean_over = len(self.codebook)
         if decoder_channels is None:
             decoder_channels = [c // 2 for c in enc_ch[1:]][::-1]
         self.decoder = UnetDecoder(enc_ch, decoder_channels)
@@ -53,7 +55,6 @@
         return feats
 
     def quantize(self, feats):
-        loss = torch.zeros(1, device=feats[0].device)
         usage = []
         levels = [i for i, vq in enumerate(self.codebook) if not isinstance(vq, _IdentityVQ)]
         vqs = [self.codebook[i] for i in levels]
@@ -66,15 +67,18 @@
                 if isinstance(feats[i], nnf.S3):
                     feats[i] = feats[i].float()
             grouped = _quantize_group(vqs, [feats[i] for i in levels]) if group else None
+        mean = getattr(grouped, "mean", None)
         grouped = dict(zip(levels, grouped)) if grouped is not None else {}
+        if mean is None:
+            loss = torch.zeros(1, device=feats[0].device)
         for i, vq in enumerate(self.codebook):
             quantize, _idx, commitment, dead = grouped[i] if i in grouped else vq(feats[i])
             feats[i] = quantize
-            if commitment is not None:
+            if commitment is not None and mean is None:
                 loss = loss + commitment
             if dead is not None:
                 usage.append(dead.detach())
-        return feats, loss / len(feats), usage
+        return feats, (loss / len(feats) if mean is None else mean), usage
 
     def decode(self, feats):
         decoder_out = self.decoder(*feats)
diff --git a/vq_seg_amd/vector_quantizer/vq_img.py b/vq_seg_amd/vector_quantizer/vq_img.py
--- a/vq_seg_amd/vector_quantizer/vq_img.py
+++ b/vq_seg_amd/vector_quantizer/vq_img.py
@@ -46,10 +46,14 @@
 class _VQGroupFunction(torch.autograd.Function):
 
     @staticmethod
-    def forward(ctx, training, weights, n, fans, *tensors):
+    def forward(ctx, training, weights, n, fans, n_feats, *tensors):
         rows, codebooks, prepared = tensors[:n], tensors[n:2 * n], tensors[2 * n:3 * n]
         ctx.fans = fans
-        outs = _hip.vq_forward_group(list(rows), list(codebooks), list(prepared), training, weights)
+        ctx.n_feats = n_feats
+        outs = _hip.vq_forward_group(list(rows), list(codebooks), list(prepared), training, weights, n_feats=n_feats)
+        if n_feats is not None:
+            outs, mean = outs
+            ctx.set_materialize_grads(False)
         ctx.n, ctx.training, ctx.weights = n, bool(training), [float(w) for w in weights]
         ctx.bf16 = rows[0].dtype == torch.bfloat16
         if training:
@@ -62,18 +66,23 @@
             nondiff += [idx, dead]
             flat += [q, idx, loss, dead]
         ctx.mark_non_differentiable(*nondiff)
-        return tuple(flat)
+        return tuple(flat) if n_feats is None else tuple(flat) + (mean,)
 
     @staticmethod
     def backward(ctx, *grads):
         n = ctx.n
-        none = (None, None, None, None) + (None,) * (3 * n)
+        none = (None, None, None, None, None) + (None,) * (3 * n)
         if not ctx.training:
             return none
         saved = ctx.saved_tensors
+        g_mean = grads[4 * n] if ctx.n_feats is not None else None
+        if g_mean is not None:
+            g_mean = g_mean / ctx.n_feats
         gxs = []
         for i in range(n):
             g_quant, g_loss = grads[4 * i], grads[4 * i + 2]
+            if g_mean is not None:
+                g_loss = g_mean if g_loss is None else g_loss + g_mean
             w = ctx.weights[i]
             gl = g_loss.contiguous() if (g_loss is not None and w > 0) else None
             if ctx.bf16:
@@ -87,7 +96,7 @@
             fan = ctx.fans[i] if ctx.fans is not None else None
             if fan is not None and gxs[-1].dtype == fan[2] and nnf._fanin_deposit(fan[0], gxs[-1].reshape(fan[1])):
                 gxs[-1] = None
-        return (None, None, None, None) + tuple(gxs) + (None,) * (2 * n)
+        return (None, None, None, None, None) + tuple(gxs) + (None,) * (2 * n)
 
 
 def quantize_group(vqs, feats):
@@ -114,14 +123,27 @@
             fans.append((link, (b, h, w, c), f.dtype) if (link is not None and r.dtype == f.dtype and r.data_ptr() == f.data_ptr()) else None)
         if not any(fans):
             fans = None
-    flat = _VQGroupFunction.apply(vqs[0].training, weights, n, fans, *rows, *[vq.codebook.embedding.weight.detach() for vq in vqs],
+    n_feats = _mean_over(vqs)
+    flat = _VQGroupFunction.apply(vqs[0].training, weights, n, fans, n_feats, *rows, *[vq.codebook.embedding.weight.detach() for vq in vqs],
                                   *[vq.codebook.prepared() for vq in vqs])
-    outs = []
+    outs = _Grouped()
     for i, f in enumerate(feats):
         b, c, h, w = f.shape
         quant, idx, loss, dead = flat[4 * i:4 * i + 4]
         outs.append((quant.reshape(b, h, w, c).permute(0, 3, 1, 2), idx.reshape(b, h, w), loss, dead))
+    if n_feats is not None:
+        outs.mean = flat[4 * n]
     return outs
+
+
+class _Grouped(list):
+    mean = None
+
+
+def _mean_over(vqs):
+    over = {getattr(vq, "loss_mean_over", None) for vq in vqs}
+    n = over.pop() if len(over) == 1 else None
+    return n if n is not None and n >= len(vqs) and _hip.vq_group_tail() else None
 
 
 def _quantize_group_s3(vqs, feats):
@@ -135,9 +157,12 @@
                 not L.vqseg_vq_filter_counter_offset(b * h * w, c, cb.num_embeddings):
             return None
     rows = [f.rows.reshape(-1, 2 * f.c) for f in feats]
+    n_feats = _mean_over(vqs)
     res = _hip.vq_forward_group(rows, [vq.codebook.embedding.weight.detach() for vq in vqs], [vq.codebook.prepared() for vq in vqs],
-                                False, [float(vq.commitment_weight) for vq in vqs], s3=True)
-    outs = []
+                                False, [float(vq.commitment_weight) for vq in vqs], s3=True, n_feats=n_feats)
+    outs = _Grouped()
+    if n_feats is not None:
+        res, outs.mean = res
     for f, (quant, idx, loss, dead) in zip(feats, res):
         b, c, h, w = f.shape
         outs.append((nnf.s3_from_rows(quant.reshape(b, h, w, 2 * c), c), idx.reshape(b, h, w), loss, dead))
```
